# aleju/cat-generator

Hardware: AMD Instinct MI355X
Metric: images/sec per G+D step, G32up-c 32x32 RGB bs=128 per GPU (higher is better)
Workload: dtype f32

## Files before the change

### cat-generator_amd/csrc/common.h

```cpp
#pragma once
#include <hip/hip_runtime.h>
#include <algorithm>
#include <stdint.h>
#include <stdio.h>
#include <string.h>
#include "../../include/catgan.h"

namespace cg {

char* err_buf();
int fail(const char* fmt, ...);

inline hipStream_t S(void* s) { return reinterpret_cast<hipStream_t>(s); }

#define CG_HIP(call)                                                              \
    do {                                                                          \
        hipError_t e__ = (call);                                                  \
        if (e__ != hipSuccess)                                                    \
            return cg::fail("%s:%d %s -> %s", __FILE__, __LINE__, #call,          \
                            hipGetErrorString(e__));                              \
    } while (0)

#define CG_LAUNCH_CHECK()                                                         \
    do {                                                                          \
        hipError_t e__ = hipGetLastError();                                       \
        if (e__ != hipSuccess)                                                    \
            return cg::fail("%s:%d kernel launch -> %s", __FILE__, __LINE__,      \
                            hipGetErrorString(e__));                              \
    } while (0)

#define CG_REQUIRE(cond, ...)                                                     \
    do {                                                                          \
        if (!(cond)) return cg::fail(__VA_ARGS__);                                \
    } while (0)

constexpr int kNumCU = 256;

#ifndef CG_TIMING_PROBE
#define CG_TIMING_PROBE 0
#endif
#define CG_PROBE_HALF(fam, T) (((CG_TIMING_PROBE) & (fam)) ? ((T) + 1) / 2 : (T))
constexpr int kEwWgsPerCU = 4, kColReduceWgsPerCU = 1;

enum Opt {
    OPT_SKINNY, OPT_GEMM_BK32, OPT_WINO_BK, OPT_NN_TILE, OPT_TN_TILE, OPT_NN_SPLITS, OPT_TN_SPLITS,
    OPT_XCD_SWIZZLE, OPT_NN_GLDS, OPT_TN_GLDS, OPT_WINO_GLDS, OPT_PAD_SKIP, OPT_WINO3, OPT_WINO_DGRAD_FUSE, OPT_WINO_DGRAD_FUSE_LAUNCHES,
    OPT_WINO3_LAUNCHES, OPT_PACK_WIDE, OPT_SAMPLER_ATOMIC_LAUNCHES, OPT_COUNT
};
long opt(Opt o);
void opt_count(Opt o);

static inline int cdiv(long a, long b) { return (int)((a + b - 1) / b); }

constexpr size_t kColScratchBytes = 8u << 20;
void* col_scratch(hipStream_t stream);
hipStream_t queue_stream(hipStream_t ref, int cls, int slot);
int queue_class(hipStream_t ref, hipStream_t s);

constexpr int MAXG = 4;
constexpr int kMaxStridedGroups = 36;
template <typename T>
__device__ __forceinline__ T sel4(int i, T a, T b, T c, T d) { return i == 0 ? a : (i == 1 ? b : (i == 2 ? c : d)); }
__device__ __forceinline__ float4 ld4(const float* p) { return *reinterpret_cast<const float4*>(p); }
__device__ __forceinline__ float f4c(const float4& v, int i) { return i == 0 ? v.x : (i == 1 ? v.y : (i == 2 ? v.z : v.w)); }
template <typename T>
static inline void set4(T& p0, T& p1, T& p2, T& p3, const T* src, int n) {
    T* const dst[MAXG] = {&p0, &p1, &p2, &p3};
    for (int i = 0; i < MAXG; ++i) *dst[i] = (src && i < n) ? src[i] : nullptr;
}
__device__ __host__ __forceinline__ int phase_map(int a, int d, int pad) { return ((a + d - pad) >> 1) - ((a - pad) >> 1); }
static inline int phase_kp(int k, int pad) { return phase_map(0, k - 1, pad) + 1; }

struct WgradParts {
    const float* part;
    const float* bias_part;
    float* const* gw;
    float* const* gb;
    long gws;
    int ngroups, S, Cin, Cout, kH, kW, pad, ups;
    float scale;
};
int wgrad_finish(hipStream_t st, const WgradParts& w, bool defer);
void wgrad_discard_all();

constexpr int kSkinnyWgradBlocks = 512;
bool skinny_ok(int ngroups, int Cin, int Cout, int kH, int kW, int padH, int padW, int ups);
size_t skinny_wgrad_ws_bytes(int Cin, int Cout);
void skinny_valu_forward(hipStream_t st, const float* x, const float* w, const float* bias, float* y, int N, int H, int W, int Cin, int Cout);
void skinny_valu_wgrad(hipStream_t st, const float* x, const float* dy, float* part, float* bias_part, int N, int H, int W, int Cin, int Cout,
                       int blocks, long ppb);
bool skinny_mfma_ok(int Cin, int Cout, int H, int W);
int skinny_mfma_forward(hipStream_t st, const float* x, const float* w, const float* bias, float* y, int N, int H, int W, int Cin, int Cout);
int skinny_mfma_wgrad(hipStream_t st, const float* x, const float* dy, float* part, float* bias_part, int N, int H, int W, int Cin, int Cout,
                      int max_blocks);

bool head_wgrad_ok(int N, int T, int C, int Co);
int head_wgrad(hipStream_t st, const float* x, const float* dy, float* gw, float* gb, int N, int T, int C, int Co, float scale);
constexpr int kWino3UOffset = 9 * 64 * 64, kWino3UFloats = 16 * 64 * 64;
static inline bool wino3_layer(int Cout, int Cin, int kH, int kW) { return Cout == 64 && Cin == 64 && kH == 3 && kW == 3; }
bool wino3_geom_ok(int ngroups, int N, int H, int W, int Cin, int Cout, int kH, int kW, int padH, int padW, int ups);
int wino3_note_pack(hipStream_t st, int n, const float* const* w, float* const* wf, float* const* wb, const int* Cout, const int* Cin,
                    const int* kH, const int* kW, const int* wb_map);
int wino3_forward(hipStream_t st, int ngroups, const float* const* x, const float* const* wpk, const float* const* bias, float* const* y,
                  int N, int H, int W);

static inline int ew_grid(long n, int per_block = 256) {
    long b = (n + per_block - 1) / per_block;
    if (b < 1) b = 1;
    const long cap = (long)kNumCU * kEwWgsPerCU;
    if (b > cap) b = cap;
    return (int)b;
}

static inline bool al16(const void* p) { return ((uintptr_t)p & 15) == 0; }
template <class... P>
static inline bool vec_ok(long n, const P*... p) { return n % 4 == 0 && (al16(p) && ...); }
#define CG_EW_LAUNCH(kern, n, ...)                                                                    \
    do {                                                                                              \
        if ((n) > 0) {                                                                                \
            hipLaunchKernelGGL(kern, dim3(cg::ew_grid(n)), dim3(256), 0, cg::S(stream), __VA_ARGS__); \
            CG_LAUNCH_CHECK();                                                                        \
        }                                                                                             \
    } while (0)
#define CG_EW_LAUNCH_V(vec, kern, n, ...)                                                                                   \
    do {                                                                                                                    \
        if ((n) > 0) {                                                                                                      \
            if (vec) { constexpr int V = 4; hipLaunchKernelGGL(kern, dim3(cg::ew_grid((n) / V)), dim3(256), 0, cg::S(stream), __VA_ARGS__); } \
            else { constexpr int V = 1; hipLaunchKernelGGL(kern, dim3(cg::ew_grid((n) / V)), dim3(256), 0, cg::S(stream), __VA_ARGS__); }    \
            CG_LAUNCH_CHECK();                                                                                              \
        }                                                                                                                   \
    } while (0)

constexpr int tile_of_row_c(int l) {
    return ((l < 4 || (l >= 12 && l < 16) || (l >= 20 && l < 28)) ? 0 : 16) +
           ((l < 4 || (l >= 12 && l < 16) || (l >= 20 && l < 28)) ? (l < 4 ? l : (l < 16 ? l - 8 : l - 12)) : (l < 12 ? l - 4 : (l < 20 ? l - 8 : l - 16)));
}
__device__ __forceinline__ int tile_of_row(int l) {
    const bool ga = l < 4 || (l >= 12 && l < 16) || (l >= 20 && l < 28);
    const int rank = ga ? (l < 4 ? l : (l < 16 ? l - 8 : l - 12)) : (l < 12 ? l - 4 : (l < 20 ? l - 8 : l - 16));
    return (ga ? 0 : 16) + rank;
}
__device__ __forceinline__ void wino3_pack_item(const float* __restrict__ w, float* uf, float* ub, int idx) {
    constexpr int C = 64;
    const int co = idx / C, ci = idx % C;
    const float G[4][3] = {{1.f, 0.f, 0.f}, {.5f, .5f, .5f}, {.5f, -.5f, .5f}, {0.f, 0.f, 1.f}};
    for (int flip = 0; flip < 2; ++flip) {
        float* U = flip ? ub : uf;
        if (!U) continue;
        float g[3][3];
        for (int a = 0; a < 3; ++a)
            for (int b = 0; b < 3; ++b) g[a][b] = flip ? w[((long)ci * C + co) * 9 + (2 - a) * 3 + (2 - b)] : w[((long)co * C + ci) * 9 + a * 3 + b];
        float t[4][3];
        for (int i = 0; i < 4; ++i)
            for (int b = 0; b < 3; ++b) t[i][b] = G[i][0] * g[0][b] + G[i][1] * g[1][b] + G[i][2] * g[2][b];
        for (int i = 0; i < 4; ++i)
            for (int k = 0; k < 4; ++k)
                U[(((long)(i * 4 + k) * (C / 4) + ci / 4) * C + co) * 4 + (ci & 3)] = t[i][0] * G[k][0] + t[i][1] * G[k][1] + t[i][2] * G[k][2];
    }
}
__device__ __forceinline__ float u01(uint64_t seed, uint64_t ctr) {
    uint64_t z = seed + (ctr + 1) * 0x9E3779B97F4A7C15ull;
    z = (z ^ (z >> 30)) * 0xBF58476D1CE4E5B9ull;
    z = (z ^ (z >> 27)) * 0x94D049BB133111EBull;
    z = z ^ (z >> 31);
    return (float)(z >> 40) * (1.0f / 16777216.0f);
}
__device__ __forceinline__ float wave_sum(float v) {
#pragma unroll
    for (int off = 32; off > 0; off >>= 1) v += __shfl_down(v, off, 64);
    return v;
}
__device__ __forceinline__ double wave_sum(double v) {
#pragma unroll
    for (int off = 32; off > 0; off >>= 1) v += __shfl_down(v, off, 64);
    return v;
}

#ifndef CG_COL_HANDOVER
#define CG_COL_HANDOVER 3
#endif
__device__ __forceinline__ void st_agent(double* p, double v) {
#if CG_COL_HANDOVER == 4
    const unsigned long long old = __hip_atomic_exchange((unsigned long long*)p, (unsigned long long)__double_as_longlong(v),
                                                         __ATOMIC_RELAXED, __HIP_MEMORY_SCOPE_AGENT);
    asm volatile("" ::"v"(old));
#else
    __hip_atomic_store(p, v, __ATOMIC_RELAXED, __HIP_MEMORY_SCOPE_AGENT);
#endif
}
__device__ __forceinline__ double ld_agent(const double* p) {
#if CG_COL_HANDOVER == 4
    unsigned long long zero = 0ull;
    asm volatile("" : "+v"(zero));
    return __longlong_as_double((long long)__hip_atomic_fetch_or((unsigned long long*)const_cast<double*>(p), zero, __ATOMIC_RELAXED,
                                                                 __HIP_MEMORY_SCOPE_AGENT));
#else
    return __hip_atomic_load(const_cast<double*>(p), __ATOMIC_RELAXED, __HIP_MEMORY_SCOPE_AGENT);
#endif
}

__device__ __forceinline__ bool last_block_arrives(unsigned* counter, unsigned total) {
    __shared__ int last_flag;
#if CG_COL_HANDOVER == 0
    __threadfence();
#else
    asm volatile("s_waitcnt vmcnt(0)" ::: "memory");
#endif
    __syncthreads();
    if (threadIdx.x == 0) {
#if CG_COL_HANDOVER == 3
        __builtin_amdgcn_fence(__ATOMIC_RELEASE, "agent");
#endif
        const unsigned t = __hip_atomic_fetch_add(counter, 1u, __ATOMIC_RELAXED, __HIP_MEMORY_SCOPE_AGENT);
        last_flag = (t == total - 1) ? 1 : 0;
        if (last_flag) __hip_atomic_store(counter, 0u, __ATOMIC_RELAXED, __HIP_MEMORY_SCOPE_AGENT);
    }
    __syncthreads();
#if CG_COL_HANDOVER == 0
    if (last_flag) __threadfence();
#elif CG_COL_HANDOVER == 3
    if (last_flag) __builtin_amdgcn_fence(__ATOMIC_ACQUIRE, "agent");
#endif
    return last_flag != 0;
}

struct ColTree {
    int G, ngroups;
    unsigned* counters;
    double* part;
    double* grp;
    double* extra;
};
constexpr int kColTreeMaxGroups = 32;
static inline bool col_tree_layout(char* scr, long chunks, size_t nk, size_t nextra, ColTree& t) {
    t.G = (int)std::max<long>(16, (chunks + kColTreeMaxGroups - 1) / kColTreeMaxGroups);
// ... 143 lines not shown
```

### cat-generator_amd/csrc/gemm.hip

```cpp
#include "common.h"
#include <stdlib.h>
#include <algorithm>
#include <type_traits>

using cg::f4c;
using cg::kMaxStridedGroups;
using cg::ld4;
using cg::MAXG;
using cg::phase_kp;
using cg::sel4;
using cg::set4;

namespace {

typedef float f32x16 __attribute__((ext_vector_type(16)));
typedef unsigned int u32x4 __attribute__((ext_vector_type(4)));

constexpr int BK = 16;
constexpr unsigned OOB = 0x80000000u;
#ifdef CG_TRACE
__device__ unsigned long long* g_trace;
#define CG_STAMP(slot)                                                                                                  \
    do {                                                                                                                \
        if (threadIdx.x == 0 && g_trace) {                                                                              \
// ... 1286 lines not shown
    const bool fast = (g.Cin % BK == 0) && al;
    const bool vecb = (g.Cout % 4 == 0) && alw;
    const bool bk32 = cg::opt(cg::OPT_GEMM_BK32) != 0 && (g.Cin % 32 == 0) && (p.kchunk % 32 == 0);
    if (a.xcd_swizzle & 4) {
        const int ntn = cg::cdiv(g.Cout, p.tc.bn);
        const double xb = (double)(g.M / (g.Hg * g.Wg)) * g.Hs * g.Ws * g.Cin * 4.0, wb = (double)g.Ktot * g.Cout * 4.0;
        if (!(ntn == 2 || ntn == 4 || ntn == 8) || ntn * xb + (8 / ntn) * wb >= xb + 8 * wb) a.xcd_swizzle &= ~4;
    }
    if (p.pm) {
        a.g.pmn = g.M / (g.Hg * g.Wg);
        a.g.pm_lg = ilog2_exact(a.g.pmn);
    }
    dim3 grid(cg::cdiv(g.M, p.tc.bm) * cg::cdiv(g.Cout, p.tc.bn), p.splits, g.nphase * ngroups);
    with_block_tile(p.tc, [&](auto t) {
        using T = decltype(t);
        launch_nn<T::BM, T::BN, T::WM, T::WN>(a, grid, st, fast, vecb, bk32);
    });
    CG_LAUNCH_CHECK();
    if (p.splits > 1) {
        const long PMN = (long)ngroups * g.nphase * g.M * g.Cout;
        bool v4 = g.Cout % 4 == 0 && (uintptr_t)ws % 16 == 0;
        for (int i = 0; i < ngroups; ++i)
            v4 = v4 && (uintptr_t)y[i] % 16 == 0 && (!bias || (uintptr_t)bias[i] % 16 == 0) && (!a.act || (uintptr_t)ep->y_act[i] % 16 == 0);
        if ((PMN >= 256L * 1024 || p.splits < 8) && v4)
            hipLaunchKernelGGL((nn_splitk_reduce_kernel<1, true>), dim3(cg::ew_grid(PMN / 4)), dim3(256), 0, st, a, p.splits);
        else if (PMN >= 256L * 1024 || p.splits < 8)
            hipLaunchKernelGGL(nn_splitk_reduce_kernel<1>, dim3(cg::ew_grid(PMN)), dim3(256), 0, st, a, p.splits);
        else
            hipLaunchKernelGGL(nn_splitk_reduce_kernel<8>, dim3((unsigned)cg::cdiv(PMN, 32)), dim3(256), 0, st, a, p.splits);
        CG_LAUNCH_CHECK();
    }
    return 0;
}

static int conv_geom(Geom& g, int N, int Hp, int Wp, int Cin, int Cout, int kH, int kW, int padH, int padW, int ups) {
    if (check_dims(N, Hp, Wp, Cin, Cout, kH, kW, padH, padW, ups)) return 1;
    return ups ? geom_phase_fwd(g, N, Hp, Wp, Cin, Cout, kH, padH) : geom_plain(g, N, Hp, Wp, Cin, Cout, kH, kW, padH, padW);
}

}

#ifdef CG_TRACE
extern "C" int cg_debug_set_trace(void* p) {
    unsigned long long* q = (unsigned long long*)p;
    return hipMemcpyToSymbol(HIP_SYMBOL(g_trace), &q, sizeof(q)) == hipSuccess ? 0 : 1;
}
#endif

extern "C" {

size_t cg_conv2d_workspace_bytes_grouped(int ngroups, int N, int Hp, int Wp, int Cin, int Cout, int kH, int kW, int padH,
                                         int padW, int ups) {
    Geom g;
    if (ngroups < 1 || ngroups > MAXG || conv_geom(g, N, Hp, Wp, Cin, Cout, kH, kW, padH, padW, ups)) return 0;
    return nn_ws_bytes(g, plan_nn(g, ngroups), ngroups);
}
size_t cg_conv2d_workspace_bytes(int N, int Hp, int Wp, int Cin, int Cout, int kH, int kW, int padH, int padW, int ups) {
    return cg_conv2d_workspace_bytes_grouped(1, N, Hp, Wp, Cin, Cout, kH, kW, padH, padW, ups);
}

size_t cg_conv2d_stats_rows(int N, int Hp, int Wp, int Cin, int Cout, int kH, int kW, int padH, int padW, int ups) {
    Geom g;
    if (conv_geom(g, N, Hp, Wp, Cin, Cout, kH, kW, padH, padW, ups)) return 0;
    if (cg::skinny_ok(1, Cin, Cout, kH, kW, padH, padW, ups)) return 0;
    const NNPlan p = plan_nn(g, 1, false);
    if (p.splits != 1) return 0;
    const int wm = p.tc.bn == 32 ? 4 : 2;
    return (size_t)g.nphase * cg::cdiv(g.M, p.tc.bm) * wm;
}

int cg_conv2d_forward_ex(void* stream, int ngroups, const float* const* x, const float* const* wpk, const float* const* bias,
                         float* const* y, int N, int Hp, int Wp, int Cin, int Cout, int kH, int kW, int padH, int padW,
                         int ups, int act, float slope, const float* const* alpha, float* const* y_act, float* stats,
                         void* ws, size_t ws_bytes) {
    CG_REQUIRE(x && wpk && y, "cg_conv2d_forward_ex: null pointer");
    Geom g;
    if (conv_geom(g, N, Hp, Wp, Cin, Cout, kH, kW, padH, padW, ups)) return 1;
    CG_REQUIRE(!cg::skinny_ok(ngroups, Cin, Cout, kH, kW, padH, padW, ups) || (act == 0 && !stats),
               "cg_conv2d_forward_ex: no fused epilogue on the skinny (<= 4 output planes) path");
    if (act == 0 && !stats)
        return cg_conv2d_forward_grouped(stream, ngroups, x, wpk, bias, y, N, Hp, Wp, Cin, Cout, kH, kW, padH, padW, ups, ws,
                                         ws_bytes);
    Epi ep{act, slope, alpha, y_act, stats};
    return run_nn(cg::S(stream), g, ngroups, x, wpk, bias, y, ws, ws_bytes, "cg_conv2d_forward_ex", &ep);
}

int cg_conv2d_forward_grouped(void* stream, int ngroups, const float* const* x, const float* const* wpk,
                              const float* const* bias, float* const* y, int N, int Hp, int Wp, int Cin, int Cout, int kH,
                              int kW, int padH, int padW, int ups, void* ws, size_t ws_bytes) {
    CG_REQUIRE(x && wpk && y, "cg_conv2d_forward_grouped: null pointer");
    Geom g;
    if (conv_geom(g, N, Hp, Wp, Cin, Cout, kH, kW, padH, padW, ups)) return 1;
    if (cg::skinny_ok(ngroups, Cin, Cout, kH, kW, padH, padW, ups) && x[0] && wpk[0] && y[0] && (uintptr_t)x[0] % 16 == 0 &&
        (long)N * Hp * Wp < 0x7fffffffL) {
        const float* b0 = bias ? bias[0] : nullptr;
        if (cg::opt(cg::OPT_SKINNY) == 1 && cg::skinny_mfma_ok(Cin, Cout, Hp, Wp)) {
            if (cg::skinny_mfma_forward(cg::S(stream), x[0], wpk[0], b0, y[0], N, Hp, Wp, Cin, Cout)) return 1;
        }
        else cg::skinny_valu_forward(cg::S(stream), x[0], wpk[0], b0, y[0], N, Hp, Wp, Cin, Cout);
        CG_LAUNCH_CHECK();
        return 0;
    }
    if (cg::wino3_geom_ok(ngroups, N, Hp, Wp, Cin, Cout, kH, kW, padH, padW, ups)) {
        const int rc = cg::wino3_forward(cg::S(stream), ngroups, x, wpk, bias, y, N, Hp, Wp);
        if (rc) return rc < 0 ? 1 : 0;
    }
    return run_nn(cg::S(stream), g, ngroups, x, wpk, bias, y, ws, ws_bytes, "cg_conv2d_forward_grouped");
}

int cg_conv2d_forward(void* stream, const float* x, const float* wpk, const float* bias, float* y, int N, int Hp, int Wp,
                      int Cin, int Cout, int kH, int kW, int padH, int padW, int ups, void* ws, size_t ws_bytes) {
    return cg_conv2d_forward_grouped(stream, 1, &x, &wpk, bias ? &bias : nullptr, &y, N, Hp, Wp, Cin, Cout, kH, kW, padH, padW,
                                     ups, ws, ws_bytes);
}

size_t cg_conv2d_dgrad_ups2_workspace_bytes(int N, int Hp, int Wp, int Cin, int Cout, int k, int pad) {
    Geom g;
    if (check_dims(N, Hp, Wp, Cin, Cout, k, k, pad, pad, 1)) return 0;
    if (geom_phase_dgrad(g, N, Hp, Wp, Cin, Cout, k, pad)) return 0;
    return nn_ws_bytes(g, plan_nn(g, 1), 1);
}

int cg_conv2d_dgrad_ups2(void* stream, const float* dy, const float* wb_ph, float* dx_lo, int N, int Hp, int Wp, int Cin,
                         int Cout, int k, int pad, void* ws, size_t ws_bytes) {
    CG_REQUIRE(dy && wb_ph && dx_lo, "cg_conv2d_dgrad_ups2: null pointer");
    Geom g;
    if (check_dims(N, Hp, Wp, Cin, Cout, k, k, pad, pad, 1)) return 1;
    if (geom_phase_dgrad(g, N, Hp, Wp, Cin, Cout, k, pad)) return 1;
    return run_nn(cg::S(stream), g, 1, &dy, &wb_ph, nullptr, &dx_lo, ws, ws_bytes, "cg_conv2d_dgrad_ups2");
}

static size_t wgrad_ws_bytes_groups(int ngroups, int maxg, int N, int Hp, int Wp, int Cin, int Cout, int kH, int kW, int padH, int padW, int ups) {
    Geom g;
    if (ngroups < 1 || ngroups > maxg || conv_geom(g, N, Hp, Wp, Cin, Cout, kH, kW, padH, padW, ups)) return 0;
    const size_t reg = tn_ws_bytes(g, plan_tn(g, ngroups), ngroups);
    return cg::skinny_ok(ngroups, Cin, Cout, kH, kW, padH, padW, ups) ? std::max(reg, cg::skinny_wgrad_ws_bytes(Cin, Cout)) : reg;
}
size_t cg_conv2d_wgrad_workspace_bytes_grouped(int ngroups, int N, int Hp, int Wp, int Cin, int Cout, int kH, int kW,
                                               int padH, int padW, int ups) {
    return wgrad_ws_bytes_groups(ngroups, MAXG, N, Hp, Wp, Cin, Cout, kH, kW, padH, padW, ups);
}
size_t cg_conv2d_wgrad_workspace_bytes_strided(int ngroups, int N, int Hp, int Wp, int Cin, int Cout, int kH, int kW,
                                               int padH, int padW, int ups) {
    return wgrad_ws_bytes_groups(ngroups, kMaxStridedGroups, N, Hp, Wp, Cin, Cout, kH, kW, padH, padW, ups);
}
size_t cg_conv2d_wgrad_workspace_bytes(int N, int Hp, int Wp, int Cin, int Cout, int kH, int kW, int padH, int padW,
                                       int ups) {
    return cg_conv2d_wgrad_workspace_bytes_grouped(1, N, Hp, Wp, Cin, Cout, kH, kW, padH, padW, ups);
}

namespace {
int wgrad_impl(void* stream, int ngroups, const float* const* x, const float* const* dy, float* const* gw, float* const* gb, int N,
               int Hp, int Wp, int Cin, int Cout, int kH, int kW, int padH, int padW, int ups, float scale, void* ws, size_t ws_bytes,
               bool defer, long xgs = 0, long dgs = 0, long gws = 0, bool gemm_only = false);
}

int cg_conv2d_wgrad_grouped(void* stream, int ngroups, const float* const* x, const float* const* dy, float* const* gw,
                            float* const* gb, int N, int Hp, int Wp, int Cin, int Cout, int kH, int kW, int padH, int padW,
                            int ups, float scale, void* ws, size_t ws_bytes) {
    return wgrad_impl(stream, ngroups, x, dy, gw, gb, N, Hp, Wp, Cin, Cout, kH, kW, padH, padW, ups, scale, ws, ws_bytes, false);
}

int cg_conv2d_wgrad_grouped_deferred(void* stream, int ngroups, const float* const* x, const float* const* dy, float* const* gw,
                                     float* const* gb, int N, int Hp, int Wp, int Cin, int Cout, int kH, int kW, int padH, int padW,
                                     int ups, float scale, void* ws, size_t ws_bytes) {
    return wgrad_impl(stream, ngroups, x, dy, gw, gb, N, Hp, Wp, Cin, Cout, kH, kW, padH, padW, ups, scale, ws, ws_bytes, true);
}

int cg_conv2d_wgrad_strided(void* stream, int ngroups, const float* x, long x_stride, const float* dy, long dy_stride, float* gw,
                            long gw_stride, int N, int Hp, int Wp, int Cin, int Cout, int kH, int kW, int padH, int padW, int ups,
                            float scale, void* ws, size_t ws_bytes) {
    CG_REQUIRE(x && dy && gw && x_stride > 0 && dy_stride > 0 && gw_stride > 0, "cg_conv2d_wgrad_strided: bad arguments");
    CG_REQUIRE(ngroups >= 1 && ngroups <= kMaxStridedGroups, "cg_conv2d_wgrad_strided: 1..%d groups per launch", kMaxStridedGroups);
    return wgrad_impl(stream, ngroups, &x, &dy, &gw, nullptr, N, Hp, Wp, Cin, Cout, kH, kW, padH, padW, ups, scale, ws, ws_bytes, false,
                      x_stride, dy_stride, gw_stride);
}

int cg_conv2d_wgrad_gemm(void* stream, const float* x, const float* dy, int N, int Hp, int Wp, int Cin, int Cout, int kH, int kW, int padH,
                         int padW, int ups, void* ws, size_t ws_bytes) {
    CG_REQUIRE(x && dy && ws, "cg_conv2d_wgrad_gemm: null pointer");
    CG_REQUIRE(!cg::skinny_ok(1, Cin, Cout, kH, kW, padH, padW, ups), "cg_conv2d_wgrad_gemm: this geometry runs the skinny kernel, not the GEMM");
    float* gw = (float*)ws;
    return wgrad_impl(stream, 1, &x, &dy, &gw, nullptr, N, Hp, Wp, Cin, Cout, kH, kW, padH, padW, ups, 1.f, ws, ws_bytes, false, 0, 0, 0, true);
}

namespace {
void launch_tn_tile(const TNArgs& a, const TileCfg& tc, bool tng, dim3 grid, hipStream_t st, bool veca, bool vecb) {
    with_block_tile(tc, [&](auto t) {
        using T = decltype(t);
        if (tng) launch_tng<T::BM, T::BN, T::WM, T::WN>(a, grid, st);
        else launch_tn<T::BM, T::BN, T::WM, T::WN>(a, grid, st, veca, vecb);
    });
}

int wgrad_impl(void* stream, int ngroups, const float* const* x, const float* const* dy, float* const* gw, float* const* gb, int N,
               int Hp, int Wp, int Cin, int Cout, int kH, int kW, int padH, int padW, int ups, float scale, void* ws, size_t ws_bytes,
               bool defer, long xgs, long dgs, long gws_, bool gemm_only) {
    CG_REQUIRE(x && dy && gw, "cg_conv2d_wgrad: null pointer");
    const bool strided = xgs != 0;
    CG_REQUIRE(ngroups >= 1 && ngroups <= (strided ? kMaxStridedGroups : MAXG), "cg_conv2d_wgrad: 1..%d groups per launch", strided ? kMaxStridedGroups : MAXG);
    CG_REQUIRE(!strided || (!gb && !defer), "cg_conv2d_wgrad: strided groups carry no bias gradient and are not deferred");
    TNArgs a;
    memset(&a, 0, sizeof(a));
    if (conv_geom(a.g, N, Hp, Wp, Cin, Cout, kH, kW, padH, padW, ups)) return 1;
    const Geom& g = a.g;
    if (!strided && cg::skinny_ok(ngroups, Cin, Cout, kH, kW, padH, padW, ups) && x[0] && dy[0] && gw[0] && (uintptr_t)x[0] % 16 == 0 && ws &&
        ws_bytes >= cg::skinny_wgrad_ws_bytes(Cin, Cout) && (long)N * Hp * Wp < 0x7fffffffL) {
        hipStream_t st = cg::S(stream);
        const long npix = (long)N * Hp * Wp;
        const long ppb = (npix + cg::kSkinnyWgradBlocks - 1) / cg::kSkinnyWgradBlocks;
        int blocks = (int)((npix + ppb - 1) / ppb);
        float* part = (float*)ws;
        float* bpart = part + (size_t)cg::kSkinnyWgradBlocks * 9 * Cin * Cout;
        float* gb0 = gb ? gb[0] : nullptr;
        if (cg::opt(cg::OPT_SKINNY) == 1 && cg::skinny_mfma_ok(Cin, Cout, Hp, Wp)) {
            blocks = cg::skinny_mfma_wgrad(st, x[0], dy[0], part, gb0 ? bpart : nullptr, N, Hp, Wp, Cin, Cout, cg::kSkinnyWgradBlocks / 2);
            if (blocks < 0) return 1;
        }
        else cg::skinny_valu_wgrad(st, x[0], dy[0], part, gb0 ? bpart : nullptr, N, Hp, Wp, Cin, Cout, blocks, ppb);
        CG_LAUNCH_CHECK();
        const cg::WgradParts parts{part, gb0 ? bpart : nullptr, gw, gb, 0, 1, blocks, Cin, Cout, 3, 3, 1, 0, scale};
        return cg::wgrad_finish(st, parts, defer);
    }
    if (!strided && !gemm_only && ngroups == 1 && !ups && kH == Hp && kW == Wp && padH == 0 && padW == 0 && cg::opt(cg::OPT_PAD_SKIP) > 0 &&
        cg::opt(cg::OPT_TN_GLDS) && cg::head_wgrad_ok(N, kH * kW, Cin, Cout) && x[0] && dy[0] && gw[0] && (uintptr_t)x[0] % 16 == 0 &&
        (uintptr_t)dy[0] % 16 == 0 && (uintptr_t)gw[0] % 4 == 0)
        return cg::head_wgrad(cg::S(stream), x[0], dy[0], gw[0], gb ? gb[0] : nullptr, N, kH * kW, Cin, Cout, scale) != 0;
    TNPlan p = plan_tn(g, ngroups);
    const size_t need = tn_ws_bytes(g, p, ngroups);
    CG_REQUIRE(ws && ws_bytes >= need, "cg_conv2d_wgrad: workspace too small (%zu < %zu)", ws_bytes, need);
    const int nptr = strided ? 1 : ngroups;
    bool veca = Cin % 4 == 0, vecb = Cout % 4 == 0, any_gb = false;
    for (int i = 0; i < nptr; ++i) {
        CG_REQUIRE(x[i] && dy[i] && gw[i], "cg_conv2d_wgrad: null pointer (group %d)", i);
        veca = veca && ((uintptr_t)x[i] % 16 == 0);
        vecb = vecb && ((uintptr_t)dy[i] % 16 == 0);
        any_gb = any_gb || (gb && gb[i]);
    }
    if (strided) { veca = veca && xgs % 4 == 0; vecb = vecb && dgs % 4 == 0; }
    if (p.pm && !(veca && vecb)) p = plan_tn(g, ngroups, false);
    a.xgs = xgs; a.dgs = dgs;
    set4(a.x0, a.x1, a.x2, a.x3, x, nptr);
    set4(a.d0, a.d1, a.d2, a.d3, dy, nptr);
    a.ngroups = ngroups; a.part = (float*)ws; a.pchunk = p.pchunk;
    a.xcd_swizzle = (int)cg::opt(cg::OPT_XCD_SWIZZLE);
    const int ZP = ngroups * g.nphase;
    const long wplane = (long)g.Ktot * g.Cout;
    a.bias_part = any_gb ? (float*)ws + (size_t)p.splits * ZP * wplane : nullptr;
    hipStream_t st = cg::S(stream);
    dim3 grid(cg::cdiv(g.Ktot, p.tc.bm) * cg::cdiv(g.Cout, p.tc.bn), p.splits, ZP);
    if (p.pm && veca && vecb) a.pm_n = g.M / (g.Hg * g.Wg);
    launch_tn_tile(a, p.tc, a.pm_n || tng_ok(g, p.pchunk, veca, vecb), grid, st, veca, vecb);
    CG_LAUNCH_CHECK();
    if (gemm_only) return 0;
    const cg::WgradParts parts{(const float*)ws, a.bias_part, gw, gb, strided ? gws_ : 0, ngroups, p.splits, Cin, Cout, kH, kW, padH, ups, scale};
    return cg::wgrad_finish(st, parts, defer);
}

}

int cg_conv2d_wgrad(void* stream, const float* x, const float* dy, float* gw, float* gb, int N, int Hp, int Wp, int Cin,
                    int Cout, int kH, int kW, int padH, int padW, int ups, float scale, void* ws, size_t ws_bytes) {
    CG_REQUIRE(x && dy && gw, "cg_conv2d_wgrad: null pointer");
    return cg_conv2d_wgrad_grouped(stream, 1, &x, &dy, &gw, &gb, N, Hp, Wp, Cin, Cout, kH, kW, padH, padW, ups, scale, ws,
                                   ws_bytes);
}

}
```

### cat-generator_amd/csrc/net.hip

```cpp
#include "net_plan.h"
#include "net_compiler.h"

namespace cg { extern unsigned long g_opt_epoch; }

namespace {

Net* NET(void* h) { return reinterpret_cast<Net*>(h); }

long param_numel(const Mod& m, int slot) {
    switch (m.kind) {
        case K_LINEAR: return slot == 0 ? m.ia[0] * m.ia[1] : m.ia[1];
        case K_CONV: return slot == 0 ? m.ia[0] * m.ia[1] * m.ia[2] * m.ia[3] : m.ia[1];
        case K_PRELU: return slot == 0 ? 1 : 0;
        case K_BN: return m.ia[0];
        default: return 0;
    }
}
void collect_params(Net* n, const Mod& m, vector<std::pair<float*, long>>& out) {
    if (m.gw) out.push_back({m.gw, param_numel(m, 0)});
    if (m.gb) out.push_back({m.gb, param_numel(m, 1)});
    for (int c : m.kids) collect_params(n, *n->mods[c], out);
}

int settle_allocs(Net* n) {
// ... 51 lines not shown
    for (Op& op : ops) {
        if (at++ == join_before) {
            if (n->trace) trace_note(n, "event|wait|packs|all");
            else
                for (int t = 0; t < c.pr->nstreams; ++t)
                    if (t != 1 && hipStreamWaitEvent(c.st[t], n->pack_ev, 0) != hipSuccess) { g_cur_net = nullptr; return cg::fail("cg_net: hipStreamWaitEvent failed"); }
        }
        c.cur = op.sidx;
        const int rc = op.fn(c);
        if (rc) { g_cur_net = nullptr; cg::wgrad_discard_all(); return rc; }
    }
    g_cur_net = nullptr;
    return 0;
}

int sync_packs(Net* n, Prog* pr, Run& c, int* join_before) {
    *join_before = -1;
    if (n->params_dirty) {
        for (auto& mp : n->mods) { mp->dirty_plain = true; mp->dirty_ups = true; }
        n->params_dirty = false;
    }
    void* stream = c.S(0);
    vector<const float*> w; vector<float*> wf, wb; vector<int> co, ci, kh, kw, mp_;
    vector<Mod*> ups;
    g_cur_net = n;
    for (auto& up : n->mods) {
        Mod& m = *up;
        if (!m.is_gemm()) continue;
        if (m.wf && m.dirty_plain) {
            if (!m.w) return cg::fail("cg_net: layer %d has no weight bound (cg_net_bind)", m.id);
            w.push_back(m.w); wf.push_back(m.wf); wb.push_back(m.wb);
            if (m.pk_map == 1) { co.push_back((int)m.ia[1]); ci.push_back((int)m.map_c); kh.push_back((int)m.map_h); kw.push_back((int)m.map_w); mp_.push_back(1); }
            else if (m.kind == K_LINEAR) { co.push_back((int)m.ia[1]); ci.push_back((int)m.ia[0]); kh.push_back(1); kw.push_back(1); mp_.push_back(0); }
            else { co.push_back((int)m.ia[1]); ci.push_back((int)m.ia[0]); kh.push_back((int)m.kH()); kw.push_back((int)m.kW()); mp_.push_back(0); }
            m.dirty_plain = false;
        }
        if (m.wf_ph && m.dirty_ups) ups.push_back(&m);
    }
    if (!w.empty() && n->K->pack_conv_weight_batch(stream, (int)w.size(), w.data(), wf.data(), wb.data(), co.data(), ci.data(), kh.data(), kw.data(), mp_.data())) return 1;
    auto first_op = [&](const Mod* m) { auto it = pr->ups_first_op.find(m->id); return it == pr->ups_first_op.end() ? -1 : it->second; };
    std::stable_sort(ups.begin(), ups.end(), [&](const Mod* a, const Mod* b) { return first_op(a) < first_op(b); });
    const bool can_side = n->pack_overlap && c.st[1] != c.st[0];
    bool forked = false;
    for (size_t i = 0; i < ups.size(); ++i) {
        Mod& m = *ups[i];
        const int fo = first_op(&m);
        const bool on_side = can_side && i >= 1 && fo > 0 && fo < (int)pr->fwd.size();
        if (on_side && !forked) {
            forked = true;
            if (n->trace) trace_note(n, "event|record|packs_fork|s0\nevent|wait|packs_fork|s1");
            else if (hipEventRecord(n->pack_fork_ev, c.st[0]) != hipSuccess || hipStreamWaitEvent(c.st[1], n->pack_fork_ev, 0) != hipSuccess)
                return cg::fail("cg_net: cannot fork the packing stream");
        }
        void* st = on_side ? c.S(1) : stream;
        if (n->K->pack_conv_weight_ups2(st, m.w, m.wf_ph, m.wb_ph, (int)m.ia[1], (int)m.ia[0], (int)m.kH(), (int)((m.kH() - 1) / 2))) return 1;
        if (m.wino && n->K->conv2d_ups2_wino_pack(st, m.wf_ph, m.wb_ph, m.u_fwd, m.u_bwd, (int)m.ia[1], (int)m.ia[0])) return 1;
        if (m.u22 && n->K->conv2d_ups2_wino22_pack(st, m.wf_ph, m.wb_ph, m.u22, m.u22b, (int)m.ia[1], (int)m.ia[0])) return 1;
        if (on_side && (*join_before < 0 || fo < *join_before)) *join_before = fo;
        m.dirty_ups = false;
    }
    if (forked) {
        if (n->trace) trace_note(n, "event|record|packs|s1");
        else if (hipEventRecord(n->pack_ev, c.st[1]) != hipSuccess) return cg::fail("cg_net: hipEventRecord failed");
        n->pack_inflight = true;
    } else if ((!w.empty() || !ups.empty()) && !n->trace) {
        if (hipEventRecord(n->pack_ev, c.st[0]) != hipSuccess) return cg::fail("cg_net: hipEventRecord failed");
        n->pack_inflight = true;
    }
    g_cur_net = nullptr;
    return 0;
}

std::string prog_key(Net* n, int nd, const long* dims, int fmt) {
    std::string k = std::to_string(fmt) + ":";
    for (int i = 0; i < nd; ++i) k += std::to_string(dims[i]) + "x";
    k += "|t";
    for (auto& m : n->mods) if (m->kind == K_BN || m->kind == K_SDROP || m->kind == K_DROP) k += m->train ? '1' : '0';
    k += "|w" + std::to_string(n->world) + (n->sync_bn ? "s" : "-") + (n->bucket_overlap ? "b" : "-");
    k += "|o" + std::to_string(n->overlap_groups) + std::to_string(n->defer_wgrad) + std::to_string(n->winograd) + std::to_string(n->fusion) +
         std::to_string(n->stacking) + std::to_string(n->grouped) + std::to_string(n->share_pool) + std::to_string(n->sampler_shared) +
         std::to_string(n->view_fuse) + std::to_string(n->cat_fuse) + std::to_string(n->fuse_locnet) + std::to_string(n->head_fuse) +
         std::to_string(n->wgrad_stream) + std::to_string(n->wino22) + std::to_string(n->wino_dsplit) + "m" +
         std::to_string(n->wino_min_tiles);
    return k;
}

int forward_plan(Net* n, void* stream, int nd, const long* dims, int fmt, Prog** out) {
    const std::string key = prog_key(n, nd, dims, fmt);
    auto it = n->progs.find(key);
    if (it != n->progs.end() && it->second->opt_epoch != cg::g_opt_epoch) {
        if (n->last == it->second.get()) n->last = nullptr;
        n->progs.erase(it); it = n->progs.end();
    }
    if (it == n->progs.end()) {
        std::unique_ptr<Prog> pr(new Prog());
        pr->net = n; pr->opt_epoch = cg::g_opt_epoch;
        Val in; in.none = false; in.ext = EXT_X; in.nd = nd; for (int i = 0; i < nd; ++i) in.d[i] = dims[i]; in.fmt = fmt;
        pr->in = in;
        Compiler C(n, pr.get());
        C.ops = &pr->fwd;
        Compiler::GCtx ctx{{C.rng}};
        pr->out = C.gfwd({n->mods[0].get()}, {in}, ctx)[0];
        if (C.failed) return cg::fail("%s", n->err);
        CG_REQUIRE(!pr->out.is_tab, "cg_net_forward: the root module returns a table");
        pr->out = C.materialise(pr->out);
        pr->draws = ctx.cur[0];
        if (ensure_streams(n, std::max(pr->nstreams, n->pack_overlap && pr->ups_first_op.size() >= 2 ? 2 : 1), stream)) return 1;
        if (settle_allocs(n)) return 1;
        it = n->progs.emplace(key, std::move(pr)).first;
    }
    *out = it->second.get();
    return 0;
}

void make_buckets(Net* n, Prog* pr) {
    const Mod& root = *n->mods[0];
    bool contiguous = true; float* expect = nullptr;
    for (size_t i = 0; i < root.kids.size(); ++i) {
        vector<std::pair<float*, long>> ps;
        collect_params(n, *n->mods[root.kids[i]], ps);
        long cnt = 0; for (auto& p : ps) cnt += p.second;
        if (n->mods[root.kids[i]]->is_gemm() || pr->buckets.empty()) {
            if (ps.empty() && pr->buckets.empty()) continue;
            pr->buckets.push_back({ps.empty() ? expect : ps[0].first, 0}); pr->bucket_first.push_back((int)i);
        }
        for (auto& p : ps) { if (expect && p.first != expect) contiguous = false; expect = p.first + p.second; }
        pr->buckets.back().second += cnt;
    }
    if (!contiguous) { pr->buckets.clear(); pr->bucket_first.clear(); }
    constexpr long kMinBucket = 65536;
    vector<std::pair<float*, long>> mb; vector<int> mf;
    long accn = 0;
    for (int j = (int)pr->buckets.size() - 1; j >= 0; --j) {
        accn += pr->buckets[j].second;
        if (accn >= kMinBucket || j == 0) {
            mb.insert(mb.begin(), {pr->buckets[j].first, accn}); mf.insert(mf.begin(), pr->bucket_first[j]);
            accn = 0;
        }
    }
    pr->buckets.swap(mb); pr->bucket_first.swap(mf);
}

int compile_backward(Net* n, Prog* pr, void* stream, int acc, int gy_fmt) {
    Compiler C(n, pr);
    C.ops = &pr->bwd[acc];
    C.acc_pass = acc != 0;
    pr->bwd[acc].clear();
    Mod& root = *n->mods[0];
    if (acc && n->bucket_overlap && n->world > 1 && root.kind == K_SEQ && root.kids.size() > 1 && pr->buckets.empty()) make_buckets(n, pr);
    C.bucket_done_upto = (int)root.kids.size();
    Val go = pr->out; go.ext = EXT_GY; go.off = 0; go.p = nullptr; go.fmt = gy_fmt; go.blk = 0; go.gi = go.gc = 0;
    Val gi = C.gbwd({&root}, {pr->in}, {go}, acc != 0, true)[0];
    if (C.failed) return cg::fail("%s", n->err);
    if (acc) { C.buckets_start(); C.flush_wgrad(); C.wg_join_all(); }
    CG_REQUIRE(!gi.is_tab, "cg_net_backward: the root module's gradInput is a table");
    pr->gin[acc] = gi;
    pr->have_bwd[acc] = true;
    if (ensure_streams(n, pr->nstreams, stream)) return 1;
    return settle_allocs(n);
}

void put_val(const Val& v, float* p, int fmt, float** ptr, int* nd, long* dims, int* fmtp) {
    if (ptr) *ptr = p;
    if (nd) *nd = v.nd;
    if (dims) for (int i = 0; i < 4; ++i) dims[i] = v.d[i];
    if (fmtp) *fmtp = fmt;
}

}

extern "C" {

int cg_net_create(void** net) {
    CG_REQUIRE(net, "cg_net_create: null pointer");
    Net* n = new Net();
    *net = n;
    if (const char* e = getenv("CG_NET_OPTIONS")) {
        std::string all(e);
        size_t pos = 0;
        while (pos < all.size()) {
            size_t end = all.find(',', pos);
            if (end == std::string::npos) end = all.size();
            const std::string kv = all.substr(pos, end - pos);
            const size_t eq = kv.find('=');
            if (eq == std::string::npos || eq == 0) { delete n; *net = nullptr; return cg::fail("CG_NET_OPTIONS: expected name=value, got '%s'", kv.c_str()); }
            if (cg_net_set_option(n, kv.substr(0, eq).c_str(), atol(kv.c_str() + eq + 1))) { delete n; *net = nullptr; return 1; }
            pos = end + 1;
        }
    }
    return 0;
}

int cg_net_destroy(void* net) {
    Net* n = NET(net);
    if (!n) return 0;
    for (void* p : n->owned) { if (n->trace) free(p); else (void)hipFree(p); }
    for (auto e : n->side_ev) (void)hipEventDestroy(e);
    if (n->fork_ev) (void)hipEventDestroy(n->fork_ev);
    if (n->pack_ev) { (void)hipEventDestroy(n->pack_fork_ev); (void)hipEventDestroy(n->pack_ev); }
    if (n->pair_fork_ev) { (void)hipEventDestroy(n->pair_fork_ev); (void)hipEventDestroy(n->pair_a_ev); (void)hipEventDestroy(n->pair_join_ev); }
    for (int t = 0; t < 4; ++t) if (n->wg_fork_ev[t]) { (void)hipEventDestroy(n->wg_fork_ev[t]); (void)hipEventDestroy(n->wg_join_ev[t]); }
    delete n;
    return 0;
}

int cg_net_set_option(void* net, const char* name, long value) {
    Net* n = NET(net);
    CG_REQUIRE(n && name, "cg_net_set_option: null pointer");
    struct { const char* nm; int* p; } tab[] = {
        {"overlap_groups", &n->overlap_groups}, {"defer_wgrad", &n->defer_wgrad}, {"winograd", &n->winograd}, {"share_pool", &n->share_pool},
        {"sampler_shared", &n->sampler_shared}, {"view_fuse", &n->view_fuse}, {"cat_fuse", &n->cat_fuse}, {"stacking", &n->stacking},
        {"grouped", &n->grouped}, {"fusion", &n->fusion}, {"fuse_locnet", &n->fuse_locnet}, {"pack_overlap", &n->pack_overlap},
        {"head_fuse", &n->head_fuse}, {"wgrad_stream", &n->wgrad_stream}, {"wino_dsplit", &n->wino_dsplit}};
    if (!strcmp(name, "trace")) {
        CG_REQUIRE(n->progs.empty(), "cg_net_set_option: trace must be chosen before the first pass");
        n->trace = value != 0; n->K = n->trace ? &kTraceTable : &kRealTable;
        return 0;
    }
    if (!strcmp(name, "defer_running")) { n->defer_running = value != 0; return 0; }
    if (!strcmp(name, "winograd_min_tiles")) { n->wino_min_tiles = value; return 0; }
    if (!strcmp(name, "winograd22")) { n->wino22 = (int)value & 3; return 0; }
    if (!strcmp(name, "fuse_locnet")) { n->fuse_locnet = (int)value; return 0; }
    for (auto& t : tab) if (!strcmp(name, t.nm)) { *t.p = value != 0; return 0; }
    return cg::fail("cg_net_set_option: unknown option %s", name);
}

int cg_net_set_allocator(void* net, cg_alloc_fn alloc, void* user) {
    Net* n = NET(net);
    CG_REQUIRE(n, "cg_net_set_allocator: null net");
    n->alloc_fn = alloc; n->alloc_user = user;
    return 0;
}

int cg_net_set_hook(void* net, cg_hook_fn hook, void* user) {
    Net* n = NET(net);
    CG_REQUIRE(n, "cg_net_set_hook: null net");
    n->hook = hook; n->hook_user = user;
    return 0;
}

int cg_net_set_dp(void* net, int world, int sync_bn, void* comm_bn, void* comm_grad, int bucket_overlap) {
    Net* n = NET(net);
    CG_REQUIRE(n && world >= 1, "cg_net_set_dp: bad arguments");
    n->world = world; n->sync_bn = sync_bn != 0; n->comm_bn = comm_bn; n->comm_grad = comm_grad; n->bucket_overlap = (bucket_overlap & 1) != 0;
    n->hook_too = (bucket_overlap & 2) != 0;
    return 0;
}

int cg_net_add(void* net, int parent, int kind, const long* iargs, int niargs, const float* fargs, int nfargs, int* id) {
    Net* n = NET(net);
    CG_REQUIRE(n && id, "cg_net_add: null pointer");
    CG_REQUIRE(kind >= 0 && kind < K_COUNT, "cg_net_add: unknown module kind %d", kind);
    CG_REQUIRE(niargs <= 8 && nfargs <= 4, "cg_net_add: too many arguments");
    CG_REQUIRE(parent < (int)n->mods.size(), "cg_net_add: unknown parent %d", parent);
    CG_REQUIRE((parent < 0) == n->mods.empty(), "cg_net_add: exactly the first module is the root (parent -1)");
    if (parent >= 0) CG_REQUIRE(n->mods[parent]->is_container(), "cg_net_add: parent %d is not a container", parent);
    std::unique_ptr<Mod> m(new Mod());
    m->id = (int)n->mods.size(); m->kind = kind; m->parent = parent;
    for (int i = 0; i < niargs; ++i) m->ia[i] = iargs[i];
    for (int i = 0; i < nfargs; ++i) m->fa[i] = fargs[i];
    if (kind == K_VIEW) m->ia[7] = niargs;
    if (kind == K_CONV) CG_REQUIRE(m->ia[6] <= 1 && m->ia[7] <= 1, "cg_net_add: only stride 1 convolutions are on the path");
    if (kind == K_CONCAT) CG_REQUIRE(m->ia[0] == 2, "cg_net_add: nn.Concat joins on dimension 2 (channels)");
    if (parent >= 0) n->mods[parent]->kids.push_back(m->id);
    *id = m->id;
    n->mods.push_back(std::move(m));
    n->progs.clear(); n->last = nullptr;
    return 0;
}

int cg_net_bind(void* net, int id, int slot, float* param, float* grad) {
    Net* n = NET(net);
    CG_REQUIRE(n && id >= 0 && id < (int)n->mods.size(), "cg_net_bind: unknown module %d", id);
    Mod& m = *n->mods[id];
    if (slot == 0) { m.w = param; m.gw = grad; }
    else if (slot == 1) { m.b = param; m.gb = grad; }
    else if (slot == 2) { m.rmean = param; m.rvar = grad; }
    else return cg::fail("cg_net_bind: slot %d (0 weight, 1 bias, 2 running mean / var)", slot);
    n->params_dirty = true;
    for (auto& kv : n->progs) { kv.second->buckets.clear(); kv.second->bucket_first.clear(); kv.second->have_bwd[1] = false; kv.second->bwd[1].clear(); }
    return 0;
}

int cg_net_set_training(void* net, int id, int train) {
    Net* n = NET(net);
    CG_REQUIRE(n && id < (int)n->mods.size(), "cg_net_set_training: unknown module %d", id);
    if (id < 0) for (auto& m : n->mods) m->train = train != 0;
    else n->mods[id]->train = train != 0;
    return 0;
}

int cg_net_params_changed(void* net) {
    Net* n = NET(net);
    CG_REQUIRE(n, "cg_net_params_changed: null net");
    n->params_dirty = true;
    return 0;
}

int cg_net_trace_region(void* net, const void* base, size_t bytes) {
    Net* n = NET(net);
    CG_REQUIRE(n && base, "cg_net_trace_region: null pointer");
    n->regions.push_back(Region{(const char*)base, bytes});
    return 0;
}

int cg_net_trace_take(void* net, char* out, size_t cap, size_t* len) {
    Net* n = NET(net);
// ... 168 lines not shown
```

### cat-generator_amd/csrc/net_compiler.h

```cpp
#pragma once

namespace {

struct Compiler {
    struct GCtx { vector<long> cur; };

    struct Prep { Val x; int wsel; Val out; Geo g; bool ok = true; };
    enum { W_PLAIN_F = 0, W_PH_F, W_PLAIN_B, W_PH_B, W_CANON };
    static float* wsel(const Mod* m, int sel) {
        switch (sel) {
            case W_PLAIN_F: return m->wf;
            case W_PH_F: return m->wf_ph;
            case W_PLAIN_B: return m->wb ? m->wb : m->w;
            case W_PH_B: return m->wb_ph;
            default: return m->w;
        }
    }

    Net* net;
    Prog* pr;
    vector<Op>* ops = nullptr;
    int cs = 0;
    long rng = 0;
    int dry = 0;
    bool failed = false;
    int pend[8] = {0, 0, 0, 0, 0, 0, 0, 0};
    bool wg_used[4] = {false, false, false, false};
    bool wg_unjoined[4] = {false, false, false, false};
    bool acc_pass = false;

    Compiler(Net* n, Prog* p) : net(n), pr(p) {}
    const KTable* K() const { return net->K; }
    Mod& M(int id) { return *net->mods[id]; }
    MS& S(const Mod& m) { return pr->ms[m.id]; }
    int err(const char* fmt, ...) {
        va_list ap; va_start(ap, fmt); vsnprintf(net->err, sizeof net->err, fmt, ap); va_end(ap);
        failed = true;
        return 1;
    }

    void* alloc(size_t bytes) {
        if (dry) return nullptr;
        bytes = (bytes + 255) & ~(size_t)255;
        if (bytes == 0) bytes = 256;
        void* p = nullptr;
        if (net->trace) {
            p = calloc(1, bytes);
        } else if (net->alloc_fn) {
            p = net->alloc_fn(net->alloc_user, bytes);
        } else {
            if (hipMalloc(&p, bytes) != hipSuccess || hipMemset(p, 0, bytes) != hipSuccess) p = nullptr;
            else net->fresh_allocs = true;
        }
        if (!p) { err("cg_net: allocation of %zu bytes failed", bytes); return nullptr; }
        if (!net->alloc_fn || net->trace) net->owned.push_back(p);
        net->regions.push_back(Region{(const char*)p, bytes});
        return p;
    }
    Val anon(std::initializer_list<long> dims, int fmt = PLAIN) {
        long n = 1; for (long x : dims) n *= x;
        Val v = mkval((float*)alloc((size_t)n * 4), dims, fmt);
        return v;
    }
    Val anon_like(const Val& x, int fmt) {
        Val v = x; v.p = (float*)alloc((size_t)x.numel() * 4); v.ext = 0; v.off = 0; v.fmt = fmt; v.ups = 0; v.blk = 0; v.gi = v.gc = 0;
        return v;
    }
    Val buf(const Mod& m, const std::string& role, std::initializer_list<long> dims, int fmt = PLAIN, size_t elem = 4) {
        long n = 1; for (long x : dims) n *= x;
        std::string key = role + "#" + std::to_string(n);
        MS& s = S(m);
        auto it = s.bufs.find(key);
        if (it == s.bufs.end()) {
            Val v = mkval((float*)alloc((size_t)n * elem), dims, fmt);
            s.bufs[key] = v;
            return v;
        }
        Val& b = it->second;
        Val want = mkval(nullptr, dims, fmt);
        if (!b.same_shape(want) || b.fmt != fmt) {
            const bool keep = want.nd && b.nd && want.d[0] == b.d[0];
            Val nb = reshape(b, dims, fmt, 0, keep);
            b = nb;
        }
        return b;
    }
    Val buf_like(const Mod& m, const std::string& role, const Val& like, int fmt) {
        switch (like.nd) {
            case 1: return buf(m, role, {like.d[0]}, fmt);
            case 2: return buf(m, role, {like.d[0], like.d[1]}, fmt);
            case 3: return buf(m, role, {like.d[0], like.d[1], like.d[2]}, fmt);
            default: return buf(m, role, {like.d[0], like.d[1], like.d[2], like.d[3]}, fmt);
        }
    }
    void ws_need(size_t bytes) {
        if (dry) return;
        if (bytes < 4096) bytes = 4096;
        if ((int)pr->ws.size() <= cs) { pr->ws.resize(cs + 1, nullptr); pr->ws_bytes.resize(cs + 1, 0); }
        if (pr->ws_bytes[cs] < bytes) {
            size_t nb = bytes + bytes / 4;
            pr->ws[cs] = alloc(nb);
            pr->ws_bytes[cs] = nb;
        }
    }
    template <class F> void emit(F f) {
        if (dry) return;
        ops->push_back(Op{cs, std::function<int(Run&)>(f)});
    }
    void use_stream(int sidx) { if (!dry && sidx + 1 > pr->nstreams) pr->nstreams = sidx + 1; }

    Val materialise(const Val& x) {
        if (!x.ups) return x;
        long N = x.d[0], C = x.d[1], H = x.d[2], W = x.d[3];
        Val out = anon({N, C, H, W}, NHWC);
        const KTable* k = K();
        emit([=](Run& c) { return k->upsample2x_forward(c.CS(), c.P(x), c.P(out), (int)N, (int)(H >> 1), (int)(W >> 1), (int)C); });
        return out;
    }

    Val as_nhwc(const Val& x, bool keep_ups = false) {
        if (x.fmt == NHWC) return (keep_ups || !x.ups) ? x : materialise(x);
        if (x.nd != 4) { err("cg_net: expected a 4-D feature map"); return x; }
        long N = x.d[0], C = x.d[1], H = x.d[2], W = x.d[3];
        Val out = anon({N, C, H, W}, NHWC);
        const KTable* k = K();
        emit([=](Run& c) { return k->nchw_to_nhwc(c.CS(), c.P(x), c.P(out), (int)N, (int)C, (int)H, (int)W); });
        return out;
    }
    Val as_plain(const Val& x0) {
        if (x0.fmt == PLAIN) return x0;
        Val x = materialise(x0);
        long N = x.d[0], C = x.d[1], H = x.d[2], W = x.d[3];
        Val out = anon({N, C, H, W}, PLAIN);
        const KTable* k = K();
        emit([=](Run& c) { return k->nhwc_to_nchw(c.CS(), c.P(x), c.P(out), (int)N, (int)C, (int)H, (int)W); });
        return out;
    }
    void emit_scaled_copy(const Val& dst, const Val& src, float f) {
        const KTable* k = K();
        const long n = src.phys();
        emit([=](Run& c) { return k->memcpy_d2d(c.CS(), c.P(dst), c.P(src), (size_t)n * 4); });
        emit([=](Run& c) { return k->scale(c.CS(), c.P(dst), f, n); });
    }
    Val match_fmt(const Val& g, const Val& like) {
        if (g.fmt == like.fmt) return g;
        return like.fmt == NHWC ? as_nhwc(g) : as_plain(g);
    }

    vector<Val> split(const Val& Y, int G) {
        vector<Val> out;
        const long n = Y.phys() / G, N = Y.d[0] / G;
        for (int i = 0; i < G; ++i) {
            Val v = Y.at((size_t)i * n * 4);
            v.d[0] = N; v.blk = Y.key(); v.gi = i; v.gc = G;
            out.push_back(v);
        }
        return out;
    }
    bool stacked(const vector<Val>& xs, Val* out) {
        if (xs.empty() || xs[0].is_tab || xs[0].none || !xs[0].blk || xs[0].gc != (int)xs.size()) return false;
        const Val& x0 = xs[0];
        for (size_t i = 0; i < xs.size(); ++i) {
            const Val& x = xs[i];
            if (x.is_tab || x.none || x.blk != x0.blk || x.gi != (int)i || !x.same_shape(x0) || x.fmt != x0.fmt || x.ups) return false;
        }
        if (out) {
            Val b = x0;
            b.d[0] = x0.d[0] * (long)xs.size(); b.blk = 0; b.gi = b.gc = 0;
            *out = b;
        }
        return true;
    }
    void seed_slices(const vector<Mod*>& mods, const std::string& role, const Val& shape_of, int fmt) {
        const int G = (int)mods.size();
        const long n = shape_of.numel();
        std::string key = role + "#" + std::to_string(n);
        vector<Val> cur; bool all = true;
        for (Mod* m : mods) {
            auto it = S(*m).bufs.find(key);
            if (it == S(*m).bufs.end() || !it->second.same_shape(shape_of) || it->second.fmt != fmt) { all = false; break; }
            cur.push_back(it->second);
        }
        if (all && stacked(cur, nullptr)) return;
        Val bs = shape_of; bs.d[0] *= G;
        Val block = buf_like(*mods[0], role + ".block", bs, fmt);
        vector<Val> sl = split(block, G);
        for (int i = 0; i < G; ++i) S(*mods[i]).bufs[key] = sl[i];
    }
    Val restack(const Mod& owner, vector<Val> xs, const Val& like) {
        for (auto& x : xs) x = match_fmt(x, like);
        Val bs = xs[0]; bs.d[0] *= (long)xs.size(); bs.ups = 0;
        Val block = buf_like(owner, "restack.block", bs, xs[0].fmt);
        const size_t nb = (size_t)xs[0].phys() * 4;
        const KTable* k = K();
        for (size_t i = 0; i < xs.size(); ++i) {
            Val dst = block.at(i * nb), src = xs[i];
            emit([=](Run& c) { return k->memcpy_d2d(c.CS(), c.P(dst), c.P(src), nb); });
        }
        return block;
    }

    void need_plain(Mod& m, bool map, long C = 0, long H = 0, long W = 0) {
        if (dry) return;
        const size_t n = cg_pack_conv_weight_floats((int)m.ia[1], (int)m.ia[0], (int)m.kH(), (int)m.kW());
        const long taps = map ? H * W : m.kH() * m.kW();
        const int want = map ? 1 : 0;
        if (m.pk_map == want && (!map || (m.map_c == C && m.map_h == H && m.map_w == W))) return;
        if (!m.wf) m.wf = (float*)alloc(n * 4);
        if (taps > 1 && !m.wb) m.wb = (float*)alloc(n * 4);
        if (taps <= 1) m.wb = nullptr;
        m.pk_map = want; m.map_c = C; m.map_h = H; m.map_w = W;
        m.dirty_plain = true;
    }
    void need_ups(Mod& m, bool wino) {
        if (dry) return;
        if (ops == &pr->fwd && !pr->ups_first_op.count(m.id)) pr->ups_first_op[m.id] = (int)ops->size();
        if (!m.wf_ph) {
            const size_t n = cg_pack_conv_weight_ups2_floats((int)m.ia[1], (int)m.ia[0], (int)m.kH(), (int)((m.kH() - 1) / 2));
            m.wf_ph = (float*)alloc(n * 4); m.wb_ph = (float*)alloc(n * 4);
            m.dirty_ups = true;
        }
        if (wino && !m.wino) {
            m.wino = true;
            const size_t nu = cg_conv2d_ups2_wino_u_floats((int)m.ia[0], (int)m.ia[1]);
            m.u_fwd = (float*)alloc(nu * 4); m.u_bwd = (float*)alloc(nu * 4);
            m.dirty_ups = true;
        }
    }

    static bool can_fold_ups(const Mod& m) { return m.kH() == m.kW() && m.kH() % 2 == 1 && m.padH() == m.padW() && m.padH() == (m.kH() - 1) / 2; }
    bool use_wino22(Mod& m, const Val& x) {
        if (!(net->winograd && (net->wino22 & 1) && m.kind == K_CONV && x.ups && m.kH() == 3 && m.kW() == 3 && m.padH() == 1 && m.padW() == 1)) return false;
        const long N = x.d[0], Hp = x.d[2] >> 1, Wp = x.d[3] >> 1;
        if (N * Hp * Wp / 4 < net->wino_min_tiles) return false;
        return cg_conv2d_ups2_wino22_supported((int)N, (int)Hp, (int)Wp, (int)m.ia[0], (int)m.ia[1]) != 0;
    }
    bool use_wino(Mod& m, const Val& x) {
        if (!(net->winograd && m.kind == K_CONV && x.ups && m.kH() == 5 && m.kW() == 5 && m.padH() == 2 && m.padW() == 2)) return false;
        const long N = x.d[0], Hp = x.d[2] >> 1, Wp = x.d[3] >> 1;
        if (N * Hp * Wp / 4 < net->wino_min_tiles) return false;
        return cg_conv2d_ups2_wino_supported((int)N, (int)Hp, (int)Wp, (int)m.ia[0], (int)m.ia[1], 5, 2) != 0;
    }
    static bool epilogue_ok(const Geo& g) {
        const bool skinny = g.ups == 0 && g.kH == 3 && g.kW == 3 && g.padH == 1 && g.padW == 1 && (g.Cout == 1 || g.Cout == 3) &&
                            (g.Cin == 64 || g.Cin == 128);
        return !skinny;
    }
    Prep prep_fwd(Mod& m, const Val& in) {
        Prep p;
        MS& s = S(m);
        if (m.kind == K_LINEAR) {
            Val x = in;
            const long o = m.ia[1];
            if (s.map_in && !(x.nd == 4 && x.fmt == NHWC && !x.ups && x.d[1] == s.mc && x.d[2] == s.mh && x.d[3] == s.mw)) s.map_in = false;
            if (s.map_in) {
                const long N = x.d[0];
                need_plain(m, true, s.mc, s.mh, s.mw);
                p.x = x; p.wsel = W_PLAIN_F; p.out = buf(m, "out", {N, o});
                p.g = Geo{(int)N, (int)s.mh, (int)s.mw, (int)s.mc, (int)o, (int)s.mh, (int)s.mw, 0, 0, 0};
                return p;
            }
            x = as_plain(x);
            const long N = x.d[0], i = x.numel() / x.d[0];
            need_plain(m, false);
            p.x = x; p.wsel = W_PLAIN_F; p.out = buf(m, "out", {N, o});
            p.g = Geo{(int)N, 1, 1, (int)i, (int)o, 1, 1, 0, 0, 0};
            return p;
        }
        Val x = as_nhwc(in, true);
        if (x.ups && !can_fold_ups(m)) x = materialise(x);
        const long N = x.d[0], H = x.d[2], W = x.d[3];
        const long Hp = H >> x.ups, Wp = W >> x.ups, Ho = H + 2 * m.padH() - m.kH() + 1, Wo = W + 2 * m.padW() - m.kW() + 1;
        if (x.d[1] != m.ia[0]) { err("cg_net: convolution %d got %ld input planes, expects %ld", m.id, x.d[1], m.ia[0]); }
        if (x.ups) { need_ups(m, false); p.wsel = W_PH_F; } else { need_plain(m, false); p.wsel = W_PLAIN_F; }
        p.x = x;
        p.out = buf(m, "out", {N, m.ia[1], Ho, Wo}, NHWC);
        p.g = Geo{(int)N, (int)Hp, (int)Wp, (int)m.ia[0], (int)m.ia[1], (int)m.kH(), (int)m.kW(), (int)m.padH(), (int)m.padW(), x.ups};
        return p;
    }
    Prep prep_gin(Mod& m, const Val& go) {
        Prep p;
        MS& s = S(m);
        if (m.kind == K_LINEAR) {
            Val dy = as_plain(go);
            const long N = dy.d[0], o = dy.numel() / dy.d[0], i = m.ia[0];
            p.x = dy;
            if (s.map_in) {
                p.wsel = W_PLAIN_B; p.out = buf(m, "gin", {N, s.mc, s.mh, s.mw}, NHWC);
            } else {
                p.wsel = W_CANON; p.out = buf(m, "gin", {N, i});
            }
            p.g = Geo{(int)N, 1, 1, (int)o, (int)i, 1, 1, 0, 0, 0};
            return p;
        }
        const Val& x = s.x;
        if (x.ups) { p.ok = false; return p; }
        Val dy = as_nhwc(go);
        const long N = dy.d[0], Ho = dy.d[2], Wo = dy.d[3];
        p.x = dy; p.wsel = W_PLAIN_B;
        p.out = buf(m, "gin", {N, m.ia[0], x.d[2], x.d[3]}, NHWC);
        p.g = Geo{(int)N, (int)Ho, (int)Wo, (int)m.ia[1], (int)m.ia[0], (int)m.kH(), (int)m.kW(), (int)(m.kH() - 1 - m.padH()),
                  (int)(m.kW() - 1 - m.padW()), 0};
        return p;
    }
    struct PrepAcc { Val x, dy; Geo g; };
    PrepAcc prep_acc(Mod& m, const Val& go) {
        PrepAcc p;
        MS& s = S(m);
        p.x = s.x;
        if (m.kind == K_LINEAR) {
            p.dy = as_plain(go);
            if (s.map_in) p.g = Geo{(int)p.x.d[0], (int)s.mh, (int)s.mw, (int)s.mc, (int)m.ia[1], (int)s.mh, (int)s.mw, 0, 0, 0};
            else p.g = Geo{(int)p.x.d[0], 1, 1, (int)(p.x.numel() / p.x.d[0]), (int)m.ia[1], 1, 1, 0, 0, 0};
            return p;
        }
        p.dy = as_nhwc(go);
        const Val& x = s.x;
        p.g = Geo{(int)x.d[0], (int)(x.d[2] >> x.ups), (int)(x.d[3] >> x.ups), (int)m.ia[0], (int)m.ia[1], (int)m.kH(), (int)m.kW(),
                  (int)m.padH(), (int)m.padW(), x.ups};
        return p;
    }

    bool prep_group(const vector<Mod*>& mods, const vector<Val>& ins, Prep (Compiler::*prep)(Mod&, const Val&), const char* role, bool epilogue,
                    vector<Prep>& preps) {
        const int G = (int)mods.size();
        for (int b = 0; b < G; ++b) preps.push_back((this->*prep)(*mods[b], ins[b]));
        bool ok = G <= 4, wino = false;
        for (int b = 0; b < G; ++b) {
            ok = ok && preps[b].ok && (!epilogue || epilogue_ok(preps[b].g));
            wino = wino || (ok && mods[b]->kind == K_CONV && preps[b].x.ups && use_wino(*mods[b], preps[b].x));
        }
        for (int b = 1; ok && b < G; ++b) ok = preps[b].g == preps[0].g;
        if (!ok || wino) return false;
        vector<Val> outs; for (auto& p : preps) outs.push_back(p.out);
        if (G > 1 && net->stacking && !stacked(outs, nullptr)) {
            seed_slices(mods, role, preps[0].out, preps[0].out.fmt);
            preps.clear();
            for (int b = 0; b < G; ++b) preps.push_back((this->*prep)(*mods[b], ins[b]));
        }
        return true;
    }
    struct Epi { vector<Mod*> acts; vector<Val> ya; Val part; };
    void emit_gemm(const vector<Mod*>& mods, const vector<Prep>& preps, const Epi& e, bool bias = true) {
        const KTable* k = K();
        const int G = (int)mods.size();
        const Geo g = preps[0].g;
        ws_need(cg_conv2d_workspace_bytes_grouped(G, GEO(g)));
        if (e.acts.empty() && e.part.none) {
            if (G == 1) {
                const Prep p = preps[0]; Mod* mp = mods[0];
                emit([=](Run& c) { return k->conv2d_forward(c.CS(), c.P(p.x), wsel(mp, p.wsel), bias ? mp->b : nullptr, c.P(p.out), GEO(p.g), c.W(), c.WB()); });
                return;
            }
            emit([=](Run& c) {
                const float *x[4], *w[4], *bi[4]; float* y[4];
                for (int b = 0; b < G; ++b) { x[b] = c.P(preps[b].x); w[b] = wsel(mods[b], preps[b].wsel); bi[b] = mods[b]->b; y[b] = c.P(preps[b].out); }
                return k->conv2d_forward_grouped(c.CS(), G, x, w, bias ? bi : nullptr, y, GEO(g), c.W(), c.WB());
            });
            return;
        }
        const int code = e.acts.empty() ? 0 : e.acts[0]->kind == K_PRELU ? 1 : 2;
        const float slope = code == 2 ? e.acts[0]->fa[0] : 0.f;
        const vector<Mod*> ac = e.acts; const vector<Val> ys = e.ya; const Val part = e.part;
        emit([=](Run& c) {
            const float *x[4], *w[4], *bi[4], *al[4]; float *y[4], *ya[4];
            for (int b = 0; b < G; ++b) {
                x[b] = c.P(preps[b].x); w[b] = wsel(mods[b], preps[b].wsel); bi[b] = mods[b]->b; y[b] = c.P(preps[b].out);
                if (code) { al[b] = ac[b]->w; ya[b] = c.P(ys[b]); }
            }
            return k->conv2d_forward_ex(c.CS(), G, x, w, bi, y, GEO(g), code, slope, code == 1 ? al : nullptr, code ? ya : nullptr, c.P(part), c.W(), c.WB());
        });
    }
    vector<Val> fwd_gemm(const vector<Mod*>& mods, const vector<Prep>& preps, const Epi& e) {
        emit_gemm(mods, preps, e);
        vector<Val> outs;
        for (size_t b = 0; b < mods.size(); ++b) {
            MS& s = S(*mods[b]);
            s.x = preps[b].x; s.out = preps[b].out; s.use_wino = false; s.use_wino22 = false;
            outs.push_back(preps[b].out);
        }
        return outs;
    }
    bool defer_wg() const { return net->defer_wgrad && net->fusion; }
    void emit_wgrad_group(const vector<Mod*>& mods, const vector<PrepAcc>& ap, void*& ws, size_t& ws_bytes) {
        const KTable* k = K();
        const int G = (int)mods.size();
        const Geo g = ap[0].g;
        const bool defer = defer_wg();
        const size_t need = std::max<size_t>(cg_conv2d_wgrad_workspace_bytes_grouped(G, GEO(g)), 4096);
        if (defer) {
            if (!dry && ws_bytes < need) { ws = alloc(need); ws_bytes = need; }
            if (!dry) pend[cs]++;
        } else ws_need(need);
        void* wsp = ws; const size_t wsb = ws_bytes;
        emit([=](Run& c) {
            const float *x[4], *d_[4]; float *gw[4], *gb[4];
            for (int b = 0; b < G; ++b) { x[b] = c.P(ap[b].x); d_[b] = c.P(ap[b].dy); gw[b] = mods[b]->gw; gb[b] = mods[b]->gb; }
            if (defer) return k->conv2d_wgrad_grouped_deferred(c.CS(), G, x, d_, gw, gb, GEO(g), c.scale, wsp, wsb);
            return k->conv2d_wgrad_grouped(c.CS(), G, x, d_, gw, gb, GEO(g), c.scale, c.W(), c.WB());
        });
    }

    Val fwd(Mod& m, const Val& in) {
        Val out = fwd_launches(m, in);
        S(m).out = out;
        return out;
    }
    Val fwd_launches(Mod& m, const Val& in) {
        const KTable* k = K();
        MS& s = S(m);
        switch (m.kind) {
        case K_CONCAT: return fwd_concat(m, in);
        case K_LINEAR: case K_CONV: {
            if (m.kind == K_CONV) {
                Val x = as_nhwc(in, true);
                if (use_wino(m, x)) return fwd_wino(m, x, nullptr, nullptr);
            }
            vector<Prep> preps;
            prep_group({&m}, {in}, &Compiler::prep_fwd, "out", false, preps);
            return fwd_gemm({&m}, preps, Epi())[0];
        }
        case K_PRELU: {
            Val x = materialise(in);
            Val out = buf_like(m, "out", x, x.fmt);
            const long n = x.phys(); Mod* mp = &m;
            emit([=](Run& c) { return k->prelu_forward(c.CS(), c.P(x), mp->w, c.P(out), n); });
            s.x = x;
            return out;
        }
        case K_LRELU: {
            Val x = materialise(in);
            Val out = buf_like(m, "out", x, x.fmt);
            const long n = x.phys(); const float sl = m.fa[0];
            emit([=](Run& c) { return k->leakyrelu_forward(c.CS(), c.P(x), c.P(out), sl, n); });
            s.x = x;
            return out;
        }
        case K_SIGMOID: {
            Val x = materialise(in);
            Val out = buf_like(m, "out", x, x.fmt);
            const long n = x.phys();
            emit([=](Run& c) { return k->sigmoid_forward(c.CS(), c.P(x), c.P(out), n); });
            return out;
        }
        case K_BN: {
            Val x = as_nhwc(in);
            Val out;
            if (!m.train) {
                const long N = x.d[0], C = x.d[1], H = x.d[2], W = x.d[3], Mr = N * H * W;
                out = buf(m, "out", {N, C, H, W}, NHWC);
                Mod* mp = &m; const float eps = m.fa[0];
                emit([=](Run& c) { return k->bn_forward_eval(c.CS(), c.P(x), c.P(out), mp->w, mp->b, mp->rmean, mp->rvar, Mr, (int)C, eps); });
            } else {
                out = fwd_bn_train(m, nullptr, x, Stats());
            }
            s.x = x; s.bn_fused = false;
            return out;
        }
        case K_VIEW: {
            s.skip = false;
            Val x = as_plain(in);
            const long N = x.d[0];
            s.in_nd = x.nd; for (int i = 0; i < 4; ++i) s.in_shape[i] = x.d[i];
            Val out;
            if (m.ia[7] == 3) {
                const long C = m.ia[0], H = m.ia[1], W = m.ia[2];
                out = buf(m, "out", {N, C, H, W}, NHWC);
                emit([=](Run& c) { return k->nchw_to_nhwc(c.CS(), c.P(x), c.P(out), (int)N, (int)C, (int)H, (int)W); });
            } else {
                out = reshape(x, {N, m.ia[0]}, PLAIN);
            }
            return out;
        }
        case K_COPY: return in;
        case K_TRANSPOSE: {
            Val out;
            if (m.ia[0] == 0) {
                Val x = as_nhwc(in);
                out = reshape(x, {x.d[0], x.d[2], x.d[3], x.d[1]}, PLAIN, 0, true);
            } else {
                if (in.fmt != PLAIN) err("cg_net: nn.Transpose BHWD->NCHW expects a plain tensor");
                out = reshape(in, {in.d[0], in.d[3], in.d[1], in.d[2]}, NHWC, 0, true);
            }
            return out;
        }
        case K_UPS: {
            Val x = as_nhwc(in);
            Val out = reshape(x, {x.d[0], x.d[1], 2 * x.d[2], 2 * x.d[3]}, NHWC, 1);
            return out;
        }
        case K_AVGPOOL: case K_MAXPOOL: {
            Val x = as_nhwc(in);
            const long N = x.d[0], C = x.d[1], H = x.d[2], W = x.d[3];
            Val out = buf(m, "out", {N, C, H / 2, W / 2}, NHWC);
            const bool mx = m.kind == K_MAXPOOL;
            emit([=](Run& c) { return (mx ? k->maxpool2_forward : k->avgpool2_forward)(c.CS(), c.P(x), c.P(out), (int)N, (int)H, (int)W, (int)C); });
            s.x = x;
            return out;
        }
        case K_SDROP: {
            Val x = as_nhwc(in);
            const long N = x.d[0], C = x.d[1], H = x.d[2], W = x.d[3];
            Val out = buf(m, "out", {N, C, H, W}, NHWC);
            const float p = m.fa[0];
            if (m.train) {
                Val noise = draw_masks(m, "noise", 1, N, C, &rng, false);
                emit([=](Run& c) { return k->mask_mul(c.CS(), c.P(x), c.P(noise), c.P(out), (int)N, H * W, (int)C, 1); });
                s.noise = noise;
            } else {
                emit_scaled_copy(out, x, 1.0f - p);
            }
            return out;
        }
        case K_DROP: {
            Val x = materialise(in);
            if (!m.train) return x;
            const long n = x.phys(); const float p = m.fa[0];
            Val noise = buf_like(m, "noise", x, x.fmt), out = buf_like(m, "out", x, x.fmt);
            const long off = rng; rng += n;
            emit([=](Run& c) { return k->rng_bernoulli_dev(c.CS(), c.P(noise), n, 1.0f - p, 1.0f / (1.0f - p), c.seed, c.roff + (uint64_t)off, c.rbase); });
            emit([=](Run& c) { return k->mask_mul(c.CS(), c.P(x), c.P(noise), c.P(out), 1, n, 1, 0); });
            s.noise = noise;
            return out;
        }
        case K_AFFMAT: {
            Val p = as_plain(in);
            const long N = p.d[0];
            Val out = buf(m, "out", {N, 2, 3});
            const int r = (int)m.ia[0], sc = (int)m.ia[1], tr = (int)m.ia[2];
            emit([=](Run& c) { return k->affine_matrix_forward(c.CS(), c.P(p), c.P(out), (int)N, r, sc, tr); });
            s.p = p;
            return out;
        }
        case K_AFFGRID: {
            const long N = in.d[0], H = m.ia[0], W = m.ia[1];
            Val out = buf(m, "out", {N, H, W, 2});
            Val T = in;
            emit([=](Run& c) { return k->affine_grid_forward(c.CS(), c.P(T), c.P(out), (int)N, (int)H, (int)W); });
            return out;
        }
        case K_SAMPLER: {
            if (!in.is_tab || in.tab.size() != 2) { err("cg_net: nn.BilinearSamplerBHWD expects {images, grids}"); return in; }
            Val img = in.tab[0], grid = in.tab[1];
            if (img.fmt != PLAIN || grid.fmt != PLAIN) err("cg_net: sampler inputs must be BHWD tensors");
            const long N = img.d[0], Hi = img.d[1], Wi = img.d[2], C = img.d[3], Ho = grid.d[1], Wo = grid.d[2];
            Val out = buf(m, "out", {N, Ho, Wo, C});
            emit([=](Run& c) { return k->bilinear_sampler_forward(c.CS(), c.P(img), c.P(grid), c.P(out), (int)N, (int)Hi, (int)Wi, (int)C, (int)Ho, (int)Wo); });
            s.in_img = img; s.in_grid = grid; s.has_shared = false;
            return out;
        }
// ... 315 lines not shown
            vector<Val> cur = xs;
            for (auto& colm : chain) cur = gfwd(colm, cur, ctx);
            return cur;
        }
        const int code = a0.kind == K_PRELU ? 1 : 2;
        const float slope = code == 1 ? 0.f : a0.fa[0];
        Mod& last = d0 ? *d0 : p0;
        Val out = buf(last, "out.fused", {G * N, C, H / 2, W / 2}, NHWC);
        Val mask; bool have_mask = false;
        if (d0) { mask = draw_masks(*d0, "noise.block", G, N, C, ctx.cur.data(), true); have_mask = true; }
        const int pool_max = p0.kind == K_MAXPOOL ? 1 : 0;
        vector<Mod*> ac = acts;
        emit([=](Run& c) {
            const float* al[4];
            for (int b = 0; b < G; ++b) al[b] = ac[b]->w;
            return k->act_pool2_mask_forward(c.CS(), c.P(X), c.P(out), have_mask ? c.P(mask) : nullptr, G, (int)N, (int)H, (int)W, (int)C, code, slope,
                                             code == 1 ? al : nullptr, pool_max);
        });
        vector<Val> outs = slices(out, G), masks;
        if (have_mask) masks = slices(mask, G);
        for (int b = 0; b < G; ++b) {
            MS& sa = S(*acts[b]); sa.x = xs[b]; sa.out = Val();
            MS& sp = S(*pools[b]); sp.x = Val(); sp.out = d0 ? Val() : outs[b];
            if (d0) { MS& sd = S(*drops[b]); sd.noise = masks[b]; sd.out = outs[b]; }
        }
        MS& s0 = S(a0);
        s0.fused = true; s0.fG = G; s0.fX = X; s0.fmask = have_mask ? mask : Val(); s0.fN = N; s0.fC = C; s0.fH = H; s0.fW = W;
        return outs;
    }

    Val fwd_gemm_bn_act(Mod& conv, Mod& bn, Mod& act, const Val& in) {
        const KTable* k = K();
        Val x = as_nhwc(in, true);
        const long C = conv.ia[1];
        if (C % 4 != 0) { S(bn).bn_fused = false; return fwd(act, fwd(bn, fwd(conv, in))); }
        Stats st; Val out;
        Mod* cp = &conv;
        if (use_wino(conv, x)) {
            out = fwd_wino(conv, x, &bn, &st);
        } else if (use_wino22(conv, x)) {
            Prep p = prep_fwd(conv, x);
            const long N = x.d[0], Hp = x.d[2] >> 1, Wp = x.d[3] >> 1, Ci = conv.ia[0];
            if (!dry && !conv.u22) {
                conv.u22 = (float*)alloc(cg_conv2d_ups2_wino22_u_floats((int)Ci, (int)C) * 4);
                conv.u22b = (float*)alloc(cg_conv2d_ups2_wino22_u_floats((int)Ci, (int)C) * 4);
                conv.dirty_ups = true;
            }
            out = p.out;
            Val v = buf(conv, "wino22_v", {(long)cg_conv2d_ups2_wino22_v_floats((int)N, (int)Hp, (int)Wp, (int)Ci)});
            st.rows = (long)cg_conv2d_ups2_wino_stats_rows((int)N, (int)Hp, (int)Wp, (int)Ci, (int)C);
            if (st.rows) st.part = buf(bn, "stats_part", {st.rows, 2, C});
            const Val px = p.x, part = st.part;
            emit([=](Run& c) { return k->conv2d_ups2_wino22_forward_stats(c.CS(), c.P(px), cp->u22, cp->b, c.P(out), c.P(v), (int)N, (int)Hp, (int)Wp, (int)Ci, (int)C,
                                                                         c.P(part)); });
            S(conv).x = p.x; S(conv).out = p.out; S(conv).use_wino = false; S(conv).use_wino22 = true;
        } else {
            vector<Prep> preps;
            prep_group({&conv}, {x}, &Compiler::prep_fwd, "out", false, preps);
            st.rows = epilogue_ok(preps[0].g) ? (long)cg_conv2d_stats_rows(GEO(preps[0].g)) : 0;
            if (st.rows) st.part = buf(bn, "stats_part", {st.rows, 2, C});
            out = fwd_gemm({&conv}, preps, Epi{{}, {}, st.part})[0];
        }
        Val y = fwd_bn_train(bn, &act, out, st);
        const long Mr = out.d[0] * out.d[2] * out.d[3];
        MS& sb = S(bn); sb.x = out; sb.out = Val(); sb.bn_fused = true; sb.bnM = Mr; sb.bnC = C;
        MS& sa = S(act); sa.x = Val(); sa.out = y;
        return y;
    }

    struct LocDesc { Mod *conv1, *conv2, *lin1, *lin2; int S, Cin, P, ur, us, ut, Hg, Wg; float slope; };
    bool match_loc(Mod& q, const Val& in, LocDesc& d) {
        if (!net->fuse_locnet || !net->fusion || q.kind != K_SEQ || q.kids.size() != 3) return false;
        Mod& L = M(q.kids[0]);
        static const int want[10] = {K_AVGPOOL, K_CONV, K_LRELU, K_CONV, K_LRELU, K_AVGPOOL, K_VIEW, K_LINEAR, K_LRELU, K_LINEAR};
        if (L.kind != K_SEQ || L.kids.size() != 10 || M(q.kids[1]).kind != K_AFFMAT || M(q.kids[2]).kind != K_AFFGRID) return false;
        for (int i = 0; i < 10; ++i) if (M(L.kids[i]).kind != want[i]) return false;
        if (in.is_tab || in.none || in.nd != 4 || in.fmt != NHWC || in.ups || in.d[2] != in.d[3] || in.d[2] % 4) return false;
        d.conv1 = &M(L.kids[1]); d.conv2 = &M(L.kids[3]); d.lin1 = &M(L.kids[7]); d.lin2 = &M(L.kids[9]);
        d.S = (int)(in.d[2] / 2); d.Cin = (int)in.d[1]; d.P = (int)d.lin2->ia[1];
        auto conv_ok = [](const Mod& c, long ci) { return c.ia[0] == ci && c.ia[1] == 16 && c.kW() == 3 && c.kH() == 3 && c.padW() == 1 && c.padH() == 1; };
        if (!conv_ok(*d.conv1, d.Cin) || !conv_ok(*d.conv2, 16)) return false;
        const long K3 = 16L * (d.S / 2) * (d.S / 2);
        if (M(L.kids[6]).ia[7] != 1 || M(L.kids[6]).ia[0] != K3 || d.lin1->ia[0] != K3 || d.lin1->ia[1] != 64 || d.lin2->ia[0] != 64) return false;
        d.slope = M(L.kids[2]).fa[0];
        if (M(L.kids[4]).fa[0] != d.slope || M(L.kids[8]).fa[0] != d.slope) return false;
        if (!(d.slope > 0.f)) return false;
        const Mod &am = M(q.kids[1]), &ag = M(q.kids[2]);
        d.ur = (int)am.ia[0]; d.us = (int)am.ia[1]; d.ut = (int)am.ia[2]; d.Hg = (int)ag.ia[0]; d.Wg = (int)ag.ia[1];
        if (d.P != d.ur + d.us + 2 * d.ut) return false;
        return cg_locnet_supported(d.S, d.Cin, d.P) != 0;
    }
    static void loc_weights(const vector<Mod*>& qs, Net* n, const float* w[48]) {
        for (size_t b = 0; b < qs.size(); ++b) {
            const Mod& L = *n->mods[qs[b]->kids[0]];
            const Mod *c1 = n->mods[L.kids[1]].get(), *c2 = n->mods[L.kids[3]].get(), *l1 = n->mods[L.kids[7]].get(), *l2 = n->mods[L.kids[9]].get();
            const float* v[12] = {c1->w, c1->b, c2->w, c2->b, l1->w, l1->b, l2->w, l2->b, c1->wf, c1->wb, c2->wf, c2->wb};
            for (int k = 0; k < 12; ++k) w[12 * b + k] = v[k];
        }
    }
    vector<Val> fwd_loc(const vector<Mod*>& qs, const Val& in, const LocDesc& d) {
        const KTable* k = K();
        const int G = (int)qs.size();
        Mod& q0 = *qs[0];
        const long N = in.d[0], S_ = d.S, Cin = d.Cin, K3 = 16L * (S_ / 2) * (S_ / 2);
        Val pooled = buf(q0, "loc.pooled", {G * N, Cin, S_, S_}, NHWC), h1 = buf(q0, "loc.h1", {G * N, 16, S_, S_}, NHWC),
            m2 = buf(q0, "loc.m2", {G * N, 16, S_, S_}, NHWC), h2 = buf(q0, "loc.h2", {G * N, K3}), h3 = buf(q0, "loc.h3", {G * N, 64}),
            prm = buf(q0, "loc.params", {G * N, d.P}), grid = buf(q0, "loc.grid", {G * N, d.Hg, d.Wg, 2});
        for (Mod* q : qs) {
            const Mod& L = M(q->kids[0]);
            need_plain(M(L.kids[1]), false); need_plain(M(L.kids[3]), false);
        }
        Net* n_ = net; vector<Mod*> qv = qs; const LocDesc dd = d; Val x = in;
        emit([=](Run& c) {
            const float* w[48];
            loc_weights(qv, n_, w);
            return k->locnet_forward(c.CS(), G, (int)N, c.P(x), 1, w, dd.S, dd.Cin, dd.P, dd.ur, dd.us, dd.ut, dd.slope, dd.Hg, dd.Wg, c.P(pooled), c.P(h1),
                                     c.P(m2), c.P(h2), c.P(h3), c.P(prm), c.P(grid));
        });
        vector<Val> outs = slices(grid, G);
        for (int b = 0; b < G; ++b) {
            MS& s = S(*qs[b]);
            s.out = outs[b]; s.loc_fused = true; s.locG = G; s.locN = N;
            s.ran_set = false;
        }
        MS& s0 = S(q0);
        s0.x = in;
        return outs;
    }
    vector<Val> bwd_loc(const vector<Mod*>& qs, const vector<Val>& gouts, bool acc) {
        const KTable* k = K();
        const int G = (int)qs.size();
        Mod& q0 = *qs[0];
        MS& s0 = S(q0);
        LocDesc d;
        if (!match_loc(q0, s0.x, d)) { err("cg_net: fused localisation branch lost its shape"); return gouts; }
        const long N = s0.locN, S_ = d.S, Cin = d.Cin, K3 = 16L * (S_ / 2) * (S_ / 2);
        Val GG = gather(q0, gouts, gouts[0]);
        Val pooled = buf(q0, "loc.pooled", {G * N, Cin, S_, S_}, NHWC), h1 = buf(q0, "loc.h1", {G * N, 16, S_, S_}, NHWC),
            m2 = buf(q0, "loc.m2", {G * N, 16, S_, S_}, NHWC), h2 = buf(q0, "loc.h2", {G * N, K3}), h3 = buf(q0, "loc.h3", {G * N, 64}),
            prm = buf(q0, "loc.params", {G * N, d.P});
        Val ga1 = buf(q0, "loc.ga1", {G * N, 16, S_, S_}, NHWC), ga2 = buf(q0, "loc.ga2", {G * N, 16, S_, S_}, NHWC), g3 = buf(q0, "loc.g3", {G * N, 64}),
            g4 = buf(q0, "loc.g4", {G * N, d.P}), gx = buf(q0, "loc.gx", {G * N, Cin, 2 * S_, 2 * S_}, NHWC);
        Net* n_ = net; vector<Mod*> qv = qs; const LocDesc dd = d;
        emit([=](Run& c) {
            const float* w[48];
            loc_weights(qv, n_, w);
            return k->locnet_backward(c.CS(), G, (int)N, w, dd.S, dd.Cin, dd.P, dd.ur, dd.us, dd.ut, dd.slope, dd.Hg, dd.Wg, c.P(h1), c.P(m2), c.P(h3), c.P(prm),
                                      c.P(GG), c.P(ga1), c.P(ga2), c.P(g3), c.P(g4), c.P(gx));
        });
        if (acc) {
            wg_fork();
            const long P_ = d.P;
            MS* s0p = &s0;
            wg_after_dgrad([this, G, N, S_, Cin, K3, P_, pooled, ga1, h1, ga2, h2, g3, h3, g4, qv, s0p]() {
            struct W { int li; Val x, dy; Geo g; };
            const W ws_[4] = {
                {1, pooled, ga1, Geo{(int)N, (int)S_, (int)S_, (int)Cin, 16, 3, 3, 1, 1, 0}},
                {3, h1, ga2, Geo{(int)N, (int)S_, (int)S_, 16, 16, 3, 3, 1, 1, 0}},
                {7, h2, g3, Geo{(int)N, 1, 1, (int)K3, 64, 1, 1, 0, 0, 0}},
                {9, h3, g4, Geo{(int)N, 1, 1, 64, (int)P_, 1, 1, 0, 0, 0}}};
            for (int wi = 0; wi < 4; ++wi) {
                const W& wv = ws_[wi];
                const size_t xs = (size_t)wv.x.phys() / G * 4, ds = (size_t)wv.dy.phys() / G * 4;
                vector<Mod*> lay; vector<PrepAcc> ap;
                for (int b = 0; b < G; ++b) {
                    lay.push_back(&M(M(qv[b]->kids[0]).kids[wv.li]));
                    ap.push_back(PrepAcc{wv.x.at(b * xs), wv.dy.at(b * ds), wv.g});
                }
                emit_wgrad_group(lay, ap, s0p->loc_ws[wi], s0p->loc_ws_bytes[wi]);
            }
            });
        }
        return share_gin(qs, gx);
    }

    std::string signature(const Mod& m) {
        std::string s = "(" + std::to_string(m.kind);
        for (int i = 0; i < 8; ++i) s += "," + std::to_string(m.ia[i]);
        char b[64]; snprintf(b, sizeof b, ",%a,%a,%d", m.fa[0], m.fa[1], m.train); s += b;
        for (int c : m.kids) s += signature(M(c));
        return s + ")";
    }
    vector<vector<int>> branch_groups(const Mod& q) {
        vector<std::pair<std::string, vector<int>>> by;
        for (size_t i = 0; i < q.kids.size(); ++i) {
            std::string sg = signature(M(q.kids[i]));
            bool found = false;
            for (auto& e : by) if (net->grouped && e.first == sg) { e.second.push_back((int)i); found = true; break; }
            if (!found) by.push_back({sg, {(int)i}});
        }
        vector<vector<int>> groups;
        for (auto& e : by)
            for (size_t k0 = 0; k0 < e.second.size(); k0 += 4) groups.emplace_back(e.second.begin() + k0, e.second.begin() + std::min(k0 + 4, e.second.size()));
        std::sort(groups.begin(), groups.end(), [](const vector<int>& a, const vector<int>& b) { return a[0] < b[0]; });
        return groups;
    }
    void run_groups(const vector<std::function<void()>>& thunks) {
        const bool multi = net->grouped && net->overlap_groups && thunks.size() > 1 && cs == 0 && thunks.size() <= 4;
        if (!multi) { for (auto& f : thunks) f(); return; }
        emit_event(EV_RECORD, EV_FORK, 0);
        for (size_t t = 1; t < thunks.size(); ++t) {
            const int sidx = (int)t;
            use_stream(sidx);
            cs = sidx;
            emit_event(EV_WAIT, EV_FORK, 0);
            thunks[t]();
            flush_wgrad();
            emit_event(EV_RECORD, EV_JOIN, sidx);
            cs = 0;
        }
        thunks[0]();
        for (size_t t = 1; t < thunks.size(); ++t) emit_event(EV_WAIT, EV_JOIN, (int)t);
    }
    enum { EV_RECORD = 0, EV_WAIT = 1 };
    enum { EV_FORK = 0, EV_JOIN, EV_WGFORK, EV_WGJOIN };
    void emit_event(int what, int kind, int k) {
        static const char* const names[] = {"fork", "join", "wgfork", "wgjoin"};
        const int s = cs;
        const std::string line = std::string(what == EV_RECORD ? "event|record|" : "event|wait|") + names[kind] + (kind == EV_FORK ? "" : std::to_string(k)) +
                                 "|s" + std::to_string(s);
        emit([=](Run& c) {
            Net* n = c.net;
            if (n->trace) { trace_note(n, line); return 0; }
            const hipEvent_t e = kind == EV_FORK ? n->fork_ev : kind == EV_JOIN ? n->side_ev[k - 1] : kind == EV_WGFORK ? n->wg_fork_ev[k] : n->wg_join_ev[k];
            const hipStream_t st = (hipStream_t)c.S(s);
            return (what == EV_RECORD ? hipEventRecord(e, st) : hipStreamWaitEvent(st, e, 0)) == hipSuccess ? 0 : 1;
        });
    }
    void flush_wgrad() {
        if (dry || !pend[cs]) return;
        const KTable* k = K();
        emit([=](Run& c) { return k->conv2d_wgrad_flush(c.CS()); });
        pend[cs] = 0;
    }
    bool wg_on() const { return net->wgrad_stream && net->fusion && acc_pass && !dry && cs < 4; }
    void wg_fork() {
        if (!wg_on()) return;
        emit_event(EV_RECORD, EV_WGFORK, cs);
    }
    int wg_enter() {
        const int s = cs;
        if (!wg_on()) return s;
        use_stream(4 + s);
        cs = 4 + s;
        emit_event(EV_WAIT, EV_WGFORK, s);
        wg_used[s] = true; wg_unjoined[s] = true;
        return s;
    }
    void wg_leave(int s) { cs = s; }
    void wg_before_dgrad() { wg_fork(); }
    void wg_after_dgrad(std::function<void()> f) {
        const int s_ = wg_enter(); f(); wg_leave(s_);
    }
    void wg_join_all() {
        if (dry) return;
        const int back = cs;
        for (int s = 0; s < 4; ++s) {
            if (!wg_used[s]) continue;
            cs = 4 + s;
            flush_wgrad();
            emit_event(EV_RECORD, EV_WGJOIN, s);
            cs = 0;
            emit_event(EV_WAIT, EV_WGJOIN, s);
            wg_used[s] = false;
        }
        cs = back;
    }
    long count_draws(Mod& m, const Val& in) {
        Prog tmp; tmp.net = net;
        Prog* save = pr;
        pr = &tmp; ++dry;
        GCtx ctx{{0}};
        gfwd({&m}, {in}, ctx);
        --dry; pr = save;
        return ctx.cur[0];
    }
    Val fwd_concat(Mod& q, const Val& in, Mod* drop = nullptr) {
        const KTable* k = K();
        const int nb = (int)q.kids.size();
        vector<Val> outs(nb);
        vector<long> base(nb);
        for (int i = 0; i < nb; ++i) { base[i] = rng; rng += count_draws(M(q.kids[i]), in); }
        vector<std::function<void()>> thunks;
        for (auto& idxs : branch_groups(q)) {
            thunks.push_back([&, idxs]() {
                GCtx ctx; vector<Mod*> mods; vector<Val> ins;
                for (int i : idxs) { ctx.cur.push_back(base[i]); mods.push_back(&M(q.kids[i])); ins.push_back(in); }
                vector<Val> res = gfwd(mods, ins, ctx);
                for (size_t t = 0; t < idxs.size(); ++t) outs[idxs[t]] = as_nhwc(res[t]);
            });
        }
        run_groups(thunks);
        const long N = outs[0].d[0], H = outs[0].d[2], W = outs[0].d[3];
        MS& s = S(q);
        s.sizes.clear();
        long Ct = 0; bool all4 = true;
        for (auto& o : outs) { s.sizes.push_back(o.d[1]); Ct += o.d[1]; all4 = all4 && o.d[1] % 4 == 0; }
        Val out = buf(q, "out", {N, Ct, H, W}, NHWC);
        s.cat_drop = false;
        if (drop && net->fusion && net->cat_fuse && nb <= 4 && all4) {
            vector<long> sz = s.sizes;
            MS& sd = S(*drop);
            Val noise = buf(*drop, "noise", {N, Ct});
            const long off = rng; rng += N * Ct;
            const float pdrop = drop->fa[0];
            emit([=](Run& c) {
                const float* src[4]; int cc[4];
                for (int i = 0; i < nb; ++i) { src[i] = c.P(outs[i]); cc[i] = (int)sz[i]; }
                return k->concat_channels_dropout(c.CS(), nb, src, cc, c.P(out), c.P(noise), (int)N, H * W, 1.0f - pdrop, 1.0f, c.seed, c.roff + (uint64_t)off, c.rbase);
            });
            s.cat_drop = true;
            s.out = Val();
            sd.noise = noise; sd.out = out;
            return out;
        }
        if (net->fusion && net->cat_fuse && nb <= 4 && all4) {
            vector<long> sz = s.sizes;
            emit([=](Run& c) {
                const float* src[4]; int cc[4];
                for (int i = 0; i < nb; ++i) { src[i] = c.P(outs[i]); cc[i] = (int)sz[i]; }
                return k->concat_channels(c.CS(), nb, src, cc, c.P(out), N * H * W);
            });
        } else {
            long off = 0;
            for (int i = 0; i < nb; ++i) {
                const long ci = s.sizes[i], o_ = off; Val src = outs[i];
                emit([=](Run& c) { return k->copy_channels(c.CS(), c.P(src), c.P(out), N * H * W, (int)ci, 0, (int)Ct, (int)o_, (int)ci); });
                off += ci;
            }
        }
        s.out = out;
        if (drop) return fwd(*drop, out);
        return out;
    }
    Val bwd_concat(Mod& q, const Val& in, const Val& go_, bool acc, Mod* drop = nullptr) {
        const KTable* k = K();
        const int nb = (int)q.kids.size();
        MS& s = S(q);
        const bool masked = drop && s.cat_drop;
        Val go = go_;
        if (drop && !masked) go = bwd(*drop, s.out, go_, acc);
        Val g = as_nhwc(go);
        const long N = g.d[0], Ct = g.d[1], H = g.d[2], W = g.d[3];
        vector<Val> dst(nb); vector<bool> have(nb, false);
        vector<vector<int>> groups = branch_groups(q);
        if (net->stacking) {
            for (auto& idxs : groups) {
                bool eq = idxs.size() > 1;
                for (int i : idxs) eq = eq && s.sizes[i] == s.sizes[idxs[0]];
                if (!eq) continue;
                Val block = buf(q, "gslice_block" + std::to_string(idxs[0]), {(long)idxs.size() * N, s.sizes[idxs[0]], H, W}, NHWC);
                vector<Val> sl = split(block, (int)idxs.size());
                for (size_t t = 0; t < idxs.size(); ++t) { dst[idxs[t]] = sl[t]; have[idxs[t]] = true; }
            }
        }
        bool all4 = true;
        for (int i = 0; i < nb; ++i) {
            if (!have[i]) dst[i] = buf(q, "gslice" + std::to_string(i), {N, s.sizes[i], H, W}, NHWC);
            all4 = all4 && s.sizes[i] % 4 == 0;
        }
        if (masked) {
            vector<long> sz = s.sizes;
            Val noise = S(*drop).noise;
            emit([=](Run& c) {
                float* d_[4]; int cc[4];
                for (int i = 0; i < nb; ++i) { d_[i] = c.P(dst[i]); cc[i] = (int)sz[i]; }
                return k->split_channels_masked(c.CS(), nb, c.P(g), c.P(noise), d_, cc, (int)N, H * W);
            });
            S(*drop).gin = Val();
        } else if (net->fusion && net->cat_fuse && nb <= 4 && all4) {
            vector<long> sz = s.sizes;
            emit([=](Run& c) {
                float* d_[4]; int cc[4];
                for (int i = 0; i < nb; ++i) { d_[i] = c.P(dst[i]); cc[i] = (int)sz[i]; }
                return k->split_channels(c.CS(), nb, c.P(g), d_, cc, N * H * W);
            });
        } else {
            long off = 0;
            for (int i = 0; i < nb; ++i) {
                const long ci = s.sizes[i], o_ = off; Val d_ = dst[i];
                emit([=](Run& c) { return k->copy_channels(c.CS(), c.P(g), c.P(d_), N * H * W, (int)Ct, (int)o_, (int)ci, 0, (int)ci); });
                off += ci;
            }
        }
        vector<Val> grads(nb);
        vector<std::function<void()>> thunks;
        for (auto& idxs : groups) {
            thunks.push_back([&, idxs]() {
                vector<Mod*> mods; vector<Val> ins, gs;
                for (int i : idxs) { mods.push_back(&M(q.kids[i])); ins.push_back(in); gs.push_back(dst[i]); }
                vector<Val> res = gbwd(mods, ins, gs, acc);
                for (size_t t = 0; t < idxs.size(); ++t) grads[idxs[t]] = as_nhwc(res[t]);
            });
        }
        run_groups(thunks);
        Val accv = buf_like(q, "gsum", grads[0], NHWC);
        const long n = accv.phys();
        if (net->fusion && net->cat_fuse && nb >= 2 && nb <= 4 && grads[0].phys() % 4 == 0) {
            emit([=](Run& c) {
                const float* src[4];
                for (int i = 0; i < nb; ++i) src[i] = c.P(grads[i]);
                return k->sum_n(c.CS(), nb, src, c.P(accv), n);
            });
        } else {
            Val g0 = grads[0];
// ... 587 lines not shown
```

### cat-generator_amd/csrc/runtime.hip

```cpp
#include "common.h"
#include <stdarg.h>
#include <stdlib.h>
#include <chrono>
#include <mutex>
#include <unordered_map>
#include <vector>

namespace cg {
char* err_buf() {
    static thread_local char buf[512] = {0};
    return buf;
}
int fail(const char* fmt, ...) {
    va_list ap;
    va_start(ap, fmt);
    vsnprintf(err_buf(), 512, fmt, ap);
    va_end(ap);
    return 1;
}

namespace {
struct OptDef { const char* name; long dflt; };
const OptDef kOptDefs[OPT_COUNT] = {
    {"CG_SKINNY", 1}, {"CG_GEMM_BK32", 1}, {"CG_WINO_BK", 0}, {"CG_NN_TILE", 0}, {"CG_TN_TILE", 0}, {"CG_NN_SPLITS", 0}, {"CG_TN_SPLITS", 0},
    {"CG_XCD_SWIZZLE", 7}, {"CG_NN_GLDS", 1}, {"CG_TN_GLDS", 1}, {"CG_WINO_GLDS", 1}, {"CG_PAD_SKIP", 20}, {"CG_WINO3", 1},
    {"CG_WINO_DGRAD_FUSE", 1}, {"CG_WINO_DGRAD_FUSE_LAUNCHES", 0}, {"CG_WINO3_LAUNCHES", 0}, {"CG_PACK_WIDE", 1},
    {"CG_SAMPLER_ATOMIC_LAUNCHES", 0},
};
long g_opt_val[OPT_COUNT];
int g_opt_state[OPT_COUNT];
}

void* col_scratch(hipStream_t stream) {
    constexpr int kPool = 8, kReserve = 4;
    static std::unordered_map<hipStream_t, void*> blocks;
    static std::vector<void*> pool;
    static std::mutex mu;
    std::lock_guard<std::mutex> lk(mu);
    auto it = blocks.find(stream);
    if (it != blocks.end()) return it->second;
    hipStreamCaptureStatus st = hipStreamCaptureStatusNone;
    const bool capturing = stream && hipStreamIsCapturing(stream, &st) == hipSuccess && st != hipStreamCaptureStatusNone;
    if (capturing && pool.empty()) {
        cg::fail("column reduce: no scratch block left for a stream first used inside a graph capture (run one pass on it before cg_graph_begin)");
        return nullptr;
    }
    if (!capturing && (int)pool.size() <= kReserve) {
        char* p = nullptr;
        hipStreamCaptureMode mode = hipStreamCaptureModeRelaxed;
        (void)hipThreadExchangeStreamCaptureMode(&mode);
        const bool ok = hipMalloc((void**)&p, kColScratchBytes * kPool) == hipSuccess &&
                        hipMemsetAsync(p, 0, kColScratchBytes * kPool, stream) == hipSuccess &&
                        hipStreamSynchronize(stream) == hipSuccess;
        (void)hipThreadExchangeStreamCaptureMode(&mode);
        if (!ok) {
            (void)hipGetLastError();
            if (pool.empty()) { cg::fail("column reduce: cannot allocate %zu bytes of scratch", kColScratchBytes * kPool); return nullptr; }
        } else
            for (int i = kPool - 1; i >= 0; --i) pool.insert(pool.begin(), p + (size_t)i * kColScratchBytes);
    }
    void* blk = pool.back();
    pool.pop_back();
    blocks[stream] = blk;
    return blk;
}
namespace {
__global__ void queue_probe_spin_k(unsigned long long ticks, int* sink) {
    const unsigned long long t0 = wall_clock64();
    while (wall_clock64() - t0 < ticks) { }
    if (ticks == ~0ull) *sink = 1;
}
struct QueuePool {
    std::vector<hipStream_t> s;
    std::unordered_map<hipStream_t, std::vector<int>> cls;
    std::mutex mu;
};
QueuePool& qpool() { static QueuePool p; return p; }
constexpr int kQueuePool = 24;

double probe_pair(hipStream_t a, hipStream_t b, bool both, unsigned long long ticks) {
    (void)hipStreamSynchronize(a);
    if (both) (void)hipStreamSynchronize(b);
    const auto t0 = std::chrono::steady_clock::now();
    hipLaunchKernelGGL(queue_probe_spin_k, dim3(1), dim3(64), 0, a, ticks, (int*)nullptr);
    if (both) hipLaunchKernelGGL(queue_probe_spin_k, dim3(1), dim3(64), 0, b, ticks, (int*)nullptr);
    (void)hipStreamSynchronize(a);
    if (both) (void)hipStreamSynchronize(b);
    return std::chrono::duration<double, std::milli>(std::chrono::steady_clock::now() - t0).count();
}
bool same_queue(hipStream_t a, hipStream_t b) {
    const unsigned long long ticks = 30000;
    int votes = 0;
    for (int r = 0; r < 3; ++r) {
        const double one = probe_pair(a, a, false, ticks), two = probe_pair(a, b, true, ticks);
        if (two > 1.6 * one) ++votes;
    }
    return votes >= 2;
}
}

int queue_classify(hipStream_t ref) {
    QueuePool& p = qpool();
    hipStreamCaptureStatus st = hipStreamCaptureStatusNone;
    if (ref && hipStreamIsCapturing(ref, &st) == hipSuccess && st != hipStreamCaptureStatusNone)
        return cg::fail("queue_stream: a stream's hardware queue cannot be probed inside a graph capture (run one pass on it before cg_graph_begin)");
    while ((int)p.s.size() < kQueuePool) {
        hipStream_t q;
        if (hipStreamCreateWithFlags(&q, hipStreamNonBlocking) != hipSuccess) return cg::fail("queue_stream: hipStreamCreate failed");
        p.s.push_back(q);
    }
    std::vector<int> c(p.s.size(), -1);
    std::vector<hipStream_t> rep;
    for (size_t i = 0; i < p.s.size(); ++i) {
        if (same_queue(ref, p.s[i])) { c[i] = 0; continue; }
        for (size_t k = 0; k < rep.size() && c[i] < 0; ++k)
            if (same_queue(rep[k], p.s[i])) c[i] = (int)k + 1;
        if (c[i] < 0) { rep.push_back(p.s[i]); c[i] = (int)rep.size(); }
    }
    (void)hipGetLastError();
    p.cls[ref] = c;
    return 0;
}

hipStream_t queue_stream(hipStream_t ref, int cls, int slot) {
    QueuePool& p = qpool();
    std::lock_guard<std::mutex> lk(p.mu);
    if (!p.cls.count(ref) && queue_classify(ref)) return nullptr;
    const std::vector<int>& c = p.cls[ref];
    int nclass = 0;
    for (int v : c) nclass = std::max(nclass, v + 1);
    if (nclass < 2) {
        static bool warned = false;
        if (!warned) { warned = true; fprintf(stderr, "cg: the hardware-queue probe found one queue only - side streams are plain pool streams (overlap not guaranteed)\n"); }
        return p.s[(size_t)((cls & 3) * (kQueuePool / 4) + slot % (kQueuePool / 4)) % p.s.size()];
    }
    cls = cls % nclass;
    int seen = 0;
    hipStream_t last = nullptr;
    for (size_t i = 0; i < c.size(); ++i)
        if (c[i] == cls) { last = p.s[i]; if (seen++ == slot) return p.s[i]; }
    if (last) return last;
    cg::fail("queue_stream: no pool stream on hardware queue class %d", cls);
    return nullptr;
}

int queue_class(hipStream_t ref, hipStream_t s) {
    if (s == ref) return 0;
    QueuePool& p = qpool();
    std::lock_guard<std::mutex> lk(p.mu);
    auto it = p.cls.find(ref);
    if (it == p.cls.end()) return -1;
    for (size_t i = 0; i < p.s.size(); ++i) if (p.s[i] == s) return it->second[i];
    return -1;
}

unsigned long g_opt_epoch = 1;
long opt(Opt o) {
    if (g_opt_state[o] == 0) {
        const char* e = getenv(kOptDefs[o].name);
        g_opt_val[o] = e ? atol(e) : kOptDefs[o].dflt;
        g_opt_state[o] = 1;
    }
    return g_opt_val[o];
}
void opt_count(Opt o) { opt(o); ++g_opt_val[o]; }
}

extern "C" {

int cg_abi_version(void) { return CG_TIMING_PROBE ? -1 : CG_ABI_VERSION; }
int cg_set_option(const char* name, long value) {
    CG_REQUIRE(name, "cg_set_option: null name");
    for (int i = 0; i < cg::OPT_COUNT; ++i)
        if (strcmp(name, cg::kOptDefs[i].name) == 0) {
            ++cg::g_opt_epoch;
            if (value == -1) { cg::g_opt_state[i] = 0; return 0; }
            cg::g_opt_val[i] = value; cg::g_opt_state[i] = 2;
            return 0;
        }
    return cg::fail("cg_set_option: unknown option %s", name);
}
int cg_get_option(const char* name, long* value) {
    CG_REQUIRE(name && value, "cg_get_option: null pointer");
    for (int i = 0; i < cg::OPT_COUNT; ++i)
        if (strcmp(name, cg::kOptDefs[i].name) == 0) { *value = cg::opt((cg::Opt)i); return 0; }
    return cg::fail("cg_get_option: unknown option %s", name);
}
const char* cg_last_error(void) { return cg::err_buf(); }
int cg_device_count(int* count) { CG_REQUIRE(count, "null"); CG_HIP(hipGetDeviceCount(count)); return 0; }
int cg_set_device(int device) { CG_HIP(hipSetDevice(device)); return 0; }
int cg_malloc(void** dptr, size_t bytes) { CG_REQUIRE(dptr, "null"); CG_HIP(hipMalloc(dptr, bytes)); return 0; }
int cg_free(void* dptr) { CG_HIP(hipFree(dptr)); return 0; }
int cg_memcpy_h2d(void* stream, void* dst, const void* src, size_t bytes) {
    CG_HIP(hipMemcpyAsync(dst, src, bytes, hipMemcpyHostToDevice, cg::S(stream))); return 0;
}
int cg_memcpy_d2h(void* stream, void* dst, const void* src, size_t bytes) {
    CG_HIP(hipMemcpyAsync(dst, src, bytes, hipMemcpyDeviceToHost, cg::S(stream)));
    CG_HIP(hipStreamSynchronize(cg::S(stream)));
    return 0;
}
int cg_memcpy_d2d(void* stream, void* dst, const void* src, size_t bytes) {
    CG_HIP(hipMemcpyAsync(dst, src, bytes, hipMemcpyDeviceToDevice, cg::S(stream))); return 0;
}
__global__ __launch_bounds__(256) void zero16_k(float4* __restrict__ p, long n16) {
    const float4 z = make_float4(0.f, 0.f, 0.f, 0.f);
    CG_GRID_STRIDE(i, n16) p[i] = z;
}
int cg_memset_zero(void* stream, void* dst, size_t bytes) {
    if (bytes >= (1u << 20) && (uintptr_t)dst % 16 == 0) {
        const long n16 = (long)(bytes / 16);
        CG_EW_LAUNCH(zero16_k, n16, (float4*)dst, n16);
        const size_t done = (size_t)n16 * 16;
        if (done < bytes) CG_HIP(hipMemsetAsync((char*)dst + done, 0, bytes - done, cg::S(stream)));
        return 0;
    }
    CG_HIP(hipMemsetAsync(dst, 0, bytes, cg::S(stream))); return 0;
}
int cg_stream_create(void** stream) {
    CG_REQUIRE(stream, "null");
    hipStream_t s; CG_HIP(hipStreamCreateWithFlags(&s, hipStreamNonBlocking)); *stream = (void*)s; return 0;
}
int cg_stream_on_queue(void* ref_stream, int queue_class, int slot, void** stream) {
    CG_REQUIRE(stream && queue_class >= 0 && slot >= 0, "cg_stream_on_queue: bad arguments");
    hipStream_t s = cg::queue_stream(cg::S(ref_stream), queue_class, slot);
    if (!s) return 1;
    *stream = (void*)s;
    return 0;
}
int cg_stream_destroy(void* stream) { CG_HIP(hipStreamDestroy(cg::S(stream))); return 0; }
int cg_stream_sync(void* stream) { CG_HIP(hipStreamSynchronize(cg::S(stream))); return 0; }

int cg_host_alloc(void** hptr, size_t bytes) {
    CG_REQUIRE(hptr && bytes > 0, "cg_host_alloc: bad arguments");
    CG_HIP(hipHostMalloc(hptr, bytes, hipHostMallocDefault));
    return 0;
}
int cg_host_free(void* hptr) { if (hptr) CG_HIP(hipHostFree(hptr)); return 0; }
int cg_event_create(void** event) {
    CG_REQUIRE(event, "cg_event_create: null pointer");
    hipEvent_t e; CG_HIP(hipEventCreateWithFlags(&e, hipEventDisableTiming)); *event = (void*)e; return 0;
}
int cg_event_destroy(void* event) { if (event) CG_HIP(hipEventDestroy((hipEvent_t)event)); return 0; }
int cg_event_record(void* event, void* stream) {
    CG_REQUIRE(event, "cg_event_record: null event");
    CG_HIP(hipEventRecord((hipEvent_t)event, cg::S(stream))); return 0;
}
int cg_event_sync(void* event) {
    CG_REQUIRE(event, "cg_event_sync: null event");
    CG_HIP(hipEventSynchronize((hipEvent_t)event)); return 0;
}
int cg_stream_wait_event(void* stream, void* event) {
    CG_REQUIRE(event, "cg_stream_wait_event: null event");
    CG_HIP(hipStreamWaitEvent(cg::S(stream), (hipEvent_t)event, 0)); return 0;
}
}
```

### cat-generator_amd/csrc/wgrad_finish.hip

```cpp
#include "common.h"
#include <mutex>
#include <unordered_map>
#include <vector>

namespace {

using cg::f4c;
using cg::ld4;
using cg::phase_map;
using cg::sel4;

template <bool UPS, int STEP>
__device__ __forceinline__ float fold(const float* pg, int tap, int ci, int co, int Cin, int Cout, int k, int pad, int kp, long plane, int S,
                                      long sstride, int sp0) {
    float s = 0.f;
    if (UPS) {
        const int dy = tap / k, dx = tap - dy * k;
        for (int sp = sp0; sp < S; sp += STEP)
#pragma unroll
            for (int p = 0; p < 4; ++p) {
                const int tp = phase_map(p >> 1, dy, pad) * kp + phase_map(p & 1, dx, pad);
                s += pg[(long)sp * sstride + (long)p * plane + ((long)tp * Cin + ci) * Cout + co];
            }
    } else {
        const long o = ((long)tap * Cin + ci) * Cout + co;
        constexpr int kInFlight = STEP == 8 ? 4 : 1;
#pragma unroll kInFlight
        for (int sp = sp0; sp < S; sp += STEP) s += pg[(long)sp * sstride + o];
    }
    return s;
}

__device__ __forceinline__ void add4(float4& s, const float4& p) { s.x += p.x; s.y += p.y; s.z += p.z; s.w += p.w; }
template <int STEP>
__device__ __forceinline__ float4 fold4(const float* src, int S, long sstride, int sp0) {
    float4 s = make_float4(0.f, 0.f, 0.f, 0.f);
    int sp = sp0;
    for (; sp + 3 * STEP < S; sp += 4 * STEP) {
        const float4 p0 = ld4(src + (long)sp * sstride), p1 = ld4(src + (long)(sp + STEP) * sstride);
        const float4 p2 = ld4(src + (long)(sp + 2 * STEP) * sstride), p3 = ld4(src + (long)(sp + 3 * STEP) * sstride);
        add4(s, p0); add4(s, p1); add4(s, p2); add4(s, p3);
    }
    for (; sp < S; sp += STEP) add4(s, ld4(src + (long)sp * sstride));
    return s;
}

__device__ __forceinline__ float lane_groups_sum(float (*sh)[33], int ol) {
    float t = 0.f;
#pragma unroll
    for (int r = 0; r < 8; ++r) t += sh[r][ol];
    return t;
}

__device__ __forceinline__ void bias_sum_block(float (*sh)[33], const float* bp, float* gb, int c0, int S, int P, long bsstride, int Cout, float scale) {
    const int cl = threadIdx.x & 31, ln = threadIdx.x >> 5;
    const int c = c0 + cl;
    float s = 0.f;
    if (c < Cout)
        for (int i = ln; i < S * P; i += 8) s += bp[(long)(i / P) * bsstride + (long)(i % P) * Cout + c];
    sh[ln][cl] = s;
    __syncthreads();
    if (ln == 0 && c < Cout) gb[c] += scale * lane_groups_sum(sh, cl);
}

template <bool UPS>
__global__ __launch_bounds__(256) void wgrad_reduce_kernel(const float* part, float* gw, int Cin, int Cout, int k, int KK,
                                                           int pad, int kp, int S, float scale, int CI_T, long sstride) {
    extern __shared__ float sh[];
    const int ci0 = blockIdx.x * CI_T, co0 = blockIdx.y * 32;
    const long plane = (long)(UPS ? kp * kp : KK) * Cin * Cout;
    const int n1 = KK * CI_T * 32;
    for (int idx = threadIdx.x; idx < n1; idx += 256) {
        const int co_l = idx & 31;
        const int r = idx >> 5;
        const int ci_l = r % CI_T, tap = r / CI_T;
        const int ci = ci0 + ci_l, co = co0 + co_l;
        float s = 0.f;
        if (ci < Cin && co < Cout) s = fold<UPS, 1>(part, tap, ci, co, Cin, Cout, k, pad, kp, plane, S, sstride, 0);
        sh[(ci_l * KK + tap) * 33 + co_l] = s;
    }
    __syncthreads();
    const int run = CI_T * KK;
    for (int idx = threadIdx.x; idx < n1; idx += 256) {
        const int j = idx % run, co_l = idx / run;
        const int ci_l = j / KK, tap = j - ci_l * KK;
        const int ci = ci0 + ci_l, co = co0 + co_l;
        if (ci < Cin && co < Cout) {
            float* dst = gw + ((long)co * Cin + ci) * KK + tap;
            *dst += scale * sh[j * 33 + co_l];
        }
    }
}

__global__ __launch_bounds__(256) void bias_part_reduce_kernel(const float* bp, float* gb, int S, int P, long sstride, int Cout, float scale) {
    __shared__ float sh[8][33];
    bias_sum_block(sh, bp, gb, blockIdx.x * 32, S, P, sstride, Cout, scale);
}

struct RedPtrs { float* gw0; float* gw1; float* gw2; float* gw3; float* gb0; float* gb1; float* gb2; float* gb3;
                 long gws; };
struct RedJob {
    const float* part; const float* bias_part;
    RedPtrs rp;
    long sstride, gstride, bsstride;
    int Cin, Cout, k, KK, pad, kp, S, P, ups, ngroups, wblocks, bblocks;
    int block0;
    float scale;
    int tr;
    int v4;
};
constexpr int kRedJobs = 20;
struct RedJobTable { RedJob j[kRedJobs]; int n; };

__device__ __forceinline__ float* gw_of(const RedPtrs& rp, int group) {
    return rp.gws ? rp.gw0 + (long)group * rp.gws : sel4(group, rp.gw0, rp.gw1, rp.gw2, rp.gw3);
}

template <bool UPS>
__device__ __forceinline__ void wgrad_reduce_small(float (*sh)[33], const RedJob& J, int group, int bx) {
    const int ol = threadIdx.x & 31, ln = threadIdx.x >> 5;
    const long total = (long)J.KK * J.Cin * J.Cout, plane = (long)(UPS ? J.kp * J.kp : J.KK) * J.Cin * J.Cout;
    const long i = bx * 32L + ol;
    int co = 0, ci = 0, tap = 0;
    float s = 0.f;
    if (i < total) {
        co = (int)(i % J.Cout);
        const long r = i / J.Cout;
        ci = (int)(r % J.Cin);
        tap = (int)(r / J.Cin);
        s = fold<UPS, 8>(J.part + (long)group * J.gstride, tap, ci, co, J.Cin, J.Cout, J.k, J.pad, J.kp, plane, J.S, J.sstride, ln);
    }
    sh[ln][ol] = s;
    __syncthreads();
    if (ln == 0 && i < total) gw_of(J.rp, group)[((long)co * J.Cin + ci) * J.KK + tap] += J.scale * lane_groups_sum(sh, ol);
}

__device__ __forceinline__ void wgrad_reduce_small_v4(float* shf, const RedJob& J, int group, int bx) {
    float4* sh4 = reinterpret_cast<float4*>(shf);
    const int ol = threadIdx.x & 31, ln = threadIdx.x >> 5;
    const long total = (long)J.KK * J.Cin * J.Cout;
    const long i = bx * 128L + 4 * ol;
    float4 s = make_float4(0.f, 0.f, 0.f, 0.f);
    if (i < total) s = fold4<8>(J.part + (long)group * J.gstride + i, J.S, J.sstride, ln);
    sh4[ln * 32 + ol] = s;
    __syncthreads();
    if (ln < 4 && i < total) {
        float t = 0.f;
#pragma unroll
        for (int r = 0; r < 8; ++r) t += f4c(sh4[r * 32 + ol], ln);
        const long e = i + ln;
        const int co = (int)(e % J.Cout);
        const long rr = e / J.Cout;
        const int ci = (int)(rr % J.Cin), tap = (int)(rr / J.Cin);
        gw_of(J.rp, group)[((long)co * J.Cin + ci) * J.KK + tap] += J.scale * t;
    }
}

__device__ __forceinline__ void wgrad_reduce_t_tile(float (*t)[33], const float* __restrict__ pg, float* __restrict__ gw, int ci0, int co0,
                                                    int Cin, int Cout, int S, long sstride, float scale) {
    const int tx = threadIdx.x & 31, ty = threadIdx.x >> 5;
    if ((Cout & 3) == 0 && (sstride & 3) == 0 && ((uintptr_t)pg & 15) == 0) {
        const int r = threadIdx.x >> 3, c4 = threadIdx.x & 7;
        const float4 s = fold4<1>(pg + (long)(ci0 + r) * Cout + co0 + 4 * c4, S, sstride, 0);
        t[r][4 * c4] = s.x; t[r][4 * c4 + 1] = s.y; t[r][4 * c4 + 2] = s.z; t[r][4 * c4 + 3] = s.w;
    } else
#pragma unroll
    for (int r = ty; r < 32; r += 8) t[r][tx] = fold<false, 1>(pg, 0, ci0 + r, co0 + tx, Cin, Cout, 1, 0, 0, 0, S, sstride, 0);
    __syncthreads();
#pragma unroll
    for (int r = ty; r < 32; r += 8) gw[(long)(co0 + r) * Cin + ci0 + tx] += scale * t[tx][r];
}
__global__ __launch_bounds__(256) void wgrad_reduce_t_kernel(const float* __restrict__ part, float* __restrict__ gw0, long gws, int Cin,
                                                             int Cout, int S, long sstride, long gstride, float scale) {
    __shared__ float t[32][33];
    const int group = blockIdx.z;
    wgrad_reduce_t_tile(t, part + (long)group * gstride, gw0 + (long)group * gws, blockIdx.x * 32, blockIdx.y * 32, Cin, Cout, S, sstride, scale);
}

__device__ __forceinline__ void red_block(float (*sh)[33], const RedJob& J, int group, int bx) {
    if (bx >= J.wblocks) {
        float* gb = sel4(group, J.rp.gb0, J.rp.gb1, J.rp.gb2, J.rp.gb3);
        if (gb) bias_sum_block(sh, J.bias_part + (long)group * J.P * J.Cout, gb, (bx - J.wblocks) * 32, J.S, J.P, J.bsstride, J.Cout, J.scale);
    } else if (J.tr) {
        const int nci = J.Cin / 32;
        wgrad_reduce_t_tile(sh, J.part + (long)group * J.gstride, gw_of(J.rp, group), (bx % nci) * 32, (bx / nci) * 32, J.Cin, J.Cout, J.S, J.sstride, J.scale);
    } else if (J.v4)
        wgrad_reduce_small_v4(&sh[0][0], J, group, bx);
    else if (J.ups)
        wgrad_reduce_small<true>(sh, J, group, bx);
    else
        wgrad_reduce_small<false>(sh, J, group, bx);
}

__global__ __launch_bounds__(256) void wgrad_reduce_small_kernel(RedJob J) {
    __shared__ __attribute__((aligned(16))) float sh[32][33];
    red_block(sh, J, (int)blockIdx.y, (int)blockIdx.x);
}

__global__ __launch_bounds__(256) void wgrad_reduce_batch_kernel(RedJobTable t) {
    __shared__ __attribute__((aligned(16))) float sh[32][33];
    const int b = (int)blockIdx.x;
    int ji = 0;
    for (int q = 1; q < t.n; ++q)
        if (b >= t.j[q].block0) ji = q;
    const RedJob& J = t.j[ji];
    const int per = J.wblocks + J.bblocks;
    const int group = (b - J.block0) / per;
    red_block(sh, J, group, (b - J.block0) - group * per);
}

std::mutex g_red_mu;
std::unordered_map<hipStream_t, std::vector<RedJob>> g_red_queue;

bool transposable(const cg::WgradParts& w) { return w.kH * w.kW == 1 && !w.ups && w.Cin % 32 == 0 && w.Cout % 32 == 0; }

RedJob red_job(const cg::WgradParts& w, bool defer) {
    RedJob job;
    memset(&job, 0, sizeof(job));
    const int nptr = w.gws ? 1 : w.ngroups;
    cg::set4(job.rp.gw0, job.rp.gw1, job.rp.gw2, job.rp.gw3, w.gw, nptr);
    cg::set4(job.rp.gb0, job.rp.gb1, job.rp.gb2, job.rp.gb3, w.gb, nptr);
    job.rp.gws = w.gws;
    job.part = w.part; job.bias_part = w.bias_part;
    job.Cin = w.Cin; job.Cout = w.Cout; job.k = w.kH; job.KK = w.kH * w.kW; job.pad = w.pad; job.ups = w.ups ? 1 : 0;
    job.kp = w.ups ? cg::phase_kp(w.kH, w.pad) : 0;
    job.S = w.S; job.P = w.ups ? 4 : 1; job.ngroups = w.ngroups; job.scale = w.scale;
    const long relems = (long)job.KK * w.Cin * w.Cout;
    job.gstride = (w.ups ? 4L * job.kp * job.kp : job.KK) * w.Cin * w.Cout;
    job.sstride = w.ngroups * job.gstride;
    job.bsstride = (long)w.ngroups * job.P * w.Cout;
    job.wblocks = cg::cdiv(relems, 32); job.bblocks = w.bias_part ? cg::cdiv(w.Cout, 32) : 0;
    if (defer && transposable(w)) {
        job.tr = 1; job.wblocks = (w.Cin / 32) * (w.Cout / 32);
    } else if (!w.ups && w.Cout % 4 == 0 && cg::al16(w.part) && job.sstride % 4 == 0 && job.gstride % 4 == 0) {
        job.v4 = 1; job.wblocks = cg::cdiv(relems, 128);
    }
    return job;
}

int small_reduce(hipStream_t st, bool defer, const RedJob& job) {
    if (defer) {
        std::lock_guard<std::mutex> lk(g_red_mu);
        g_red_queue[st].push_back(job);
        return 0;
    }
    hipLaunchKernelGGL(wgrad_reduce_small_kernel, dim3(job.wblocks + job.bblocks, job.ngroups), dim3(256), 0, st, job);
    CG_LAUNCH_CHECK();
    return 0;
}

}

int cg::wgrad_finish(hipStream_t st, const WgradParts& w, bool defer) {
    const RedJob job = red_job(w, defer);
    const int Cin = w.Cin, Cout = w.Cout, KK = job.KK;
    if (w.gws && transposable(w) && !w.bias_part) {
        hipLaunchKernelGGL(wgrad_reduce_t_kernel, dim3(Cin / 32, Cout / 32, w.ngroups), dim3(256), 0, st, w.part, w.gw[0], w.gws, Cin, Cout, w.S,
                           job.sstride, job.gstride, w.scale);
        CG_LAUNCH_CHECK();
        return 0;
    }
    int ci_t = KK == 1 ? 64 : 8;
    while (ci_t > 1 && (size_t)KK * ci_t * 33 * sizeof(float) > 60000) ci_t >>= 1;
    const size_t shb = (size_t)KK * ci_t * 33 * sizeof(float);
    const dim3 rgrid(cg::cdiv(Cin, ci_t), cg::cdiv(Cout, 32));
    if ((long)rgrid.x * rgrid.y < cg::kNumCU) return small_reduce(st, defer, job);
    for (int gi = 0; gi < w.ngroups; ++gi) {
        const float* pg = w.part + gi * job.gstride;
        float* gwi = w.gws ? w.gw[0] + gi * w.gws : w.gw[gi];
        hipLaunchKernelGGL(w.ups ? wgrad_reduce_kernel<true> : wgrad_reduce_kernel<false>, rgrid, dim3(256), shb, st, pg, gwi, Cin, Cout, w.kH, KK,
                           w.pad, job.kp, w.S, w.scale, ci_t, job.sstride);
        CG_LAUNCH_CHECK();
        if (w.gb && w.gb[gi]) {
            hipLaunchKernelGGL(bias_part_reduce_kernel, dim3(cg::cdiv(Cout, 32)), dim3(256), 0, st, w.bias_part + (long)gi * job.P * Cout, w.gb[gi],
                               w.S, job.P, job.bsstride, Cout, w.scale);
            CG_LAUNCH_CHECK();
        }
    }
    return 0;
}

void cg::wgrad_discard_all() {
    std::lock_guard<std::mutex> lk(g_red_mu);
    for (auto& kv : g_red_queue) kv.second.clear();
}

extern "C" {

int cg_conv2d_wgrad_pending(void* stream, int* njobs) {
    CG_REQUIRE(njobs, "cg_conv2d_wgrad_pending: null pointer");
    std::lock_guard<std::mutex> lk(g_red_mu);
    auto it = g_red_queue.find(cg::S(stream));
    *njobs = it == g_red_queue.end() ? 0 : (int)it->second.size();
    return 0;
}

int cg_conv2d_wgrad_flush(void* stream) {
    hipStream_t st = cg::S(stream);
    std::vector<RedJob> jobs;
    {
        std::lock_guard<std::mutex> lk(g_red_mu);
        auto it = g_red_queue.find(st);
        if (it == g_red_queue.end() || it->second.empty()) return 0;
        jobs.swap(it->second);
    }
    for (size_t j0 = 0; j0 < jobs.size(); j0 += kRedJobs) {
        RedJobTable t;
        memset(&t, 0, sizeof(t));
        t.n = (int)std::min<size_t>(kRedJobs, jobs.size() - j0);
        int blocks = 0;
        for (int q = 0; q < t.n; ++q) {
            t.j[q] = jobs[j0 + q];
            t.j[q].block0 = blocks;
            blocks += t.j[q].ngroups * (t.j[q].wblocks + t.j[q].bblocks);
        }
        hipLaunchKernelGGL(wgrad_reduce_batch_kernel, dim3(blocks), dim3(256), 0, st, t);
        CG_LAUNCH_CHECK();
    }
    return 0;
}

}
```

### include/catgan.h

```cpp
#ifndef CATGAN_H
#define CATGAN_H

#include <stddef.h>
#include <stdint.h>

#ifdef __cplusplus
extern "C" {
#endif

#define CG_ABI_VERSION 2

int         cg_abi_version(void);
const char* cg_last_error(void);
int cg_set_option(const char* name, long value);
int cg_get_option(const char* name, long* value);
int cg_device_count(int* count);
int cg_set_device(int device);
int cg_malloc(void** dptr, size_t bytes);
int cg_free(void* dptr);
int cg_memcpy_h2d(void* stream, void* dst, const void* src, size_t bytes);
int cg_memcpy_d2h(void* stream, void* dst, const void* src, size_t bytes);
int cg_memcpy_d2d(void* stream, void* dst, const void* src, size_t bytes);
int cg_memset_zero(void* stream, void* dst, size_t bytes);
int cg_stream_create(void** stream);
int cg_stream_on_queue(void* ref_stream, int queue_class, int slot, void** stream);
int cg_stream_destroy(void* stream);
int cg_stream_sync(void* stream);
int cg_host_alloc(void** hptr, size_t bytes);
int cg_host_free(void* hptr);
int cg_event_create(void** event);
int cg_event_destroy(void* event);
int cg_event_record(void* event, void* stream);
int cg_event_sync(void* event);
int cg_stream_wait_event(void* stream, void* event);
int cg_images_u8_to_f32(void* stream, const unsigned char* src, float* dst, long npixels, int colorspace);
int cg_images_u8_scale_to_f32(void* stream, const unsigned char* src, float* dst, int N, int Hs, int Ws, int Hd, int Wd, int colorspace);
int cg_images_u8_augment_to_f32(void* stream, const unsigned char* src, float* dst, int N, int Hs, int Ws, int Hd, int Wd,
                                int colorspace, const float* desc, float noise_std, uint64_t seed, uint64_t offset);
int cg_images_u8_gather_scale_to_f32(void* stream, const unsigned char* set, long M, const int32_t* idx, float* dst, int N, int Hs, int Ws,
                                     int Hd, int Wd, int colorspace);
int cg_images_u8_gather_augment_to_f32(void* stream, const unsigned char* set, long M, const int32_t* idx, float* dst, int N, int Hs, int Ws,
                                       int Hd, int Wd, int colorspace, const float* desc, float noise_std, uint64_t seed, uint64_t offset);
int cg_images_u8_augment_window_to_f32(void* stream, const unsigned char* src, float* dst, int N, int Hp, int Wp, int margin, int Hd, int Wd,
                                       int colorspace, const float* desc, float noise_std, uint64_t seed, uint64_t offset);
int cg_images_u8_gather_augment_window_to_f32(void* stream, const unsigned char* set, long M, const int32_t* idx, float* dst, int N, int Hp,
                                              int Wp, int margin, int Hd, int Wd, int colorspace, const float* desc, float noise_std,
                                              uint64_t seed, uint64_t offset);
int cg_faces_u8_extract(void* stream, const unsigned char* src, size_t src_bytes, const uint64_t* src_off, const int32_t* geom,
                        const float* inv, const int32_t* taps, size_t ntaps, const uint64_t* tap_off, unsigned char* dst, int N, int out,
                        void* workspace, size_t workspace_bytes);
int cg_faces_u8_extract_variants(void* stream, const unsigned char* src, size_t src_bytes, const uint64_t* src_off, const int32_t* geom,
                                 const float* inv, const int32_t* taps, size_t ntaps, const uint64_t* tap_off, int pad, int A,
                                 const float* desc, const uint64_t* bases, float noise_scale, uint64_t seed, unsigned char* dst, int N, int out,
                                 void* workspace, size_t workspace_bytes);
int cg_faces_u8_extract_padded(void* stream, const unsigned char* src, size_t src_bytes, const uint64_t* src_off, const int32_t* geom,
                               const float* inv, const int32_t* taps, size_t ntaps, const uint64_t* tap_off, const int32_t* pads,
                               unsigned char* dst, int N, int out, void* workspace, size_t workspace_bytes);
int cg_colorspace_convert(void* stream, const float* src, float* dst, long npixels, int from, int to);
size_t cg_nearest_workspace_bytes(int N, int Q, long D);
int cg_nearest_update(void* stream, const float* pool, int N, long D, const float* queries, int Q, int index0, int reset, float* best_d2,
                      int32_t* best_idx, void* workspace);

size_t cg_conv2d_workspace_bytes(int N, int Hp, int Wp, int Cin, int Cout,
                                 int kH, int kW, int padH, int padW, int ups);
int cg_conv2d_forward(void* stream, const float* x, const float* wpk, const float* bias,
                      float* y, int N, int Hp, int Wp, int Cin, int Cout,
                      int kH, int kW, int padH, int padW, int ups,
                      void* ws, size_t ws_bytes);

size_t cg_conv2d_workspace_bytes_grouped(int ngroups, int N, int Hp, int Wp, int Cin, int Cout,
                                         int kH, int kW, int padH, int padW, int ups);
int cg_conv2d_forward_grouped(void* stream, int ngroups, const float* const* x, const float* const* wpk,
                              const float* const* bias, float* const* y, int N, int Hp, int Wp, int Cin, int Cout,
                              int kH, int kW, int padH, int padW, int ups, void* ws, size_t ws_bytes);

size_t cg_conv2d_stats_rows(int N, int Hp, int Wp, int Cin, int Cout, int kH, int kW, int padH, int padW, int ups);
int cg_conv2d_forward_ex(void* stream, int ngroups, const float* const* x, const float* const* wpk,
                         const float* const* bias, float* const* y, int N, int Hp, int Wp, int Cin, int Cout,
                         int kH, int kW, int padH, int padW, int ups,
                         int act, float slope, const float* const* alpha, float* const* y_act, float* stats,
                         void* ws, size_t ws_bytes);

size_t cg_conv2d_dgrad_ups2_workspace_bytes(int N, int Hp, int Wp, int Cin, int Cout, int k, int pad);
int cg_conv2d_dgrad_ups2(void* stream, const float* dy, const float* wb_ph, float* dx_lo,
                         int N, int Hp, int Wp, int Cin, int Cout, int k, int pad,
                         void* ws, size_t ws_bytes);

size_t cg_conv2d_wgrad_workspace_bytes(int N, int Hp, int Wp, int Cin, int Cout,
                                       int kH, int kW, int padH, int padW, int ups);
int cg_conv2d_wgrad(void* stream, const float* x, const float* dy, float* gw_canonical, float* gb,
                    int N, int Hp, int Wp, int Cin, int Cout,
                    int kH, int kW, int padH, int padW, int ups, float scale,
                    void* ws, size_t ws_bytes);

size_t cg_conv2d_wgrad_workspace_bytes_grouped(int ngroups, int N, int Hp, int Wp, int Cin, int Cout,
                                               int kH, int kW, int padH, int padW, int ups);
int cg_conv2d_wgrad_grouped(void* stream, int ngroups, const float* const* x, const float* const* dy,
                            float* const* gw_canonical, float* const* gb, int N, int Hp, int Wp, int Cin, int Cout,
                            int kH, int kW, int padH, int padW, int ups, float scale, void* ws, size_t ws_bytes);
int cg_conv2d_wgrad_grouped_deferred(void* stream, int ngroups, const float* const* x, const float* const* dy,
                            float* const* gw_canonical, float* const* gb, int N, int Hp, int Wp, int Cin, int Cout,
                            int kH, int kW, int padH, int padW, int ups, float scale, void* ws, size_t ws_bytes);
int cg_conv2d_wgrad_flush(void* stream);
int cg_conv2d_wgrad_gemm(void* stream, const float* x, const float* dy, int N, int Hp, int Wp, int Cin, int Cout,
                         int kH, int kW, int padH, int padW, int ups, void* ws, size_t ws_bytes);
int cg_conv2d_wgrad_pending(void* stream, int* njobs);
size_t cg_conv2d_wgrad_workspace_bytes_strided(int ngroups, int N, int Hp, int Wp, int Cin, int Cout,
                                               int kH, int kW, int padH, int padW, int ups);
int cg_conv2d_wgrad_strided(void* stream, int ngroups, const float* x, long x_stride, const float* dy, long dy_stride,
                            float* gw_canonical, long gw_stride, int N, int Hp, int Wp, int Cin, int Cout,
                            int kH, int kW, int padH, int padW, int ups, float scale, void* ws, size_t ws_bytes);

int cg_bias_grad(void* stream, const float* dy, float* gb, long M, int C, float scale,
                 void* ws, size_t ws_bytes);

size_t cg_pack_conv_weight_floats(int Cout, int Cin, int kH, int kW);
int cg_pack_conv_weight(void* stream, const float* w_canonical, float* wf, float* wb,
                        int Cout, int Cin, int kH, int kW);
int cg_pack_conv_weight_batch(void* stream, int n, const float* const* w_canonical, float* const* wf, float* const* wb,
                              const int* Cout, const int* Cin, const int* kH, const int* kW, const int* wb_map);
int cg_pack_conv_weight_map(void* stream, const float* w_canonical, float* wf, float* wbT, int Cout, int Cin, int kH, int kW);
size_t cg_pack_conv_weight_ups2_floats(int Cout, int Cin, int k, int pad);
int cg_pack_conv_weight_ups2(void* stream, const float* w_canonical, float* wf_ph, float* wb_ph,
                             int Cout, int Cin, int k, int pad);

size_t cg_conv2d_ups2_wino_supported(int N, int Hp, int Wp, int Cin, int Cout, int k, int pad);
size_t cg_conv2d_ups2_wino_v_floats(int N, int Hp, int Wp, int C);
size_t cg_conv2d_ups2_wino_u_floats(int Cin, int Cout);
int cg_conv2d_ups2_wino_pack(void* stream, const float* wf_ph, const float* wb_ph, float* u_fwd, float* u_bwd,
                             int Cout, int Cin);
int cg_conv2d_ups2_wino_gemm(void* stream, const float* v, const float* u, const float* bias, float* y,
                             int N, int Hp, int Wp, int Cin, int Cout, int dgrad);
int cg_conv2d_ups2_wino_forward(void* stream, const float* x_lo, const float* u_fwd, const float* bias, float* y,
                                float* v, int N, int Hp, int Wp, int Cin, int Cout);
size_t cg_conv2d_ups2_wino_stats_rows(int N, int Hp, int Wp, int Cin, int Cout);
int cg_conv2d_ups2_wino_forward_stats(void* stream, const float* x_lo, const float* u_fwd, const float* bias, float* y,
                                      float* v, int N, int Hp, int Wp, int Cin, int Cout, float* stats);
size_t cg_conv2d_ups2_wino22_supported(int N, int Hp, int Wp, int Cin, int Cout);
size_t cg_conv2d_ups2_wino22_dgrad_supported(int N, int Hp, int Wp, int Cin, int Cout);
size_t cg_conv2d_ups2_wino22_v_floats(int N, int Hp, int Wp, int Cin);
size_t cg_conv2d_ups2_wino22_u_floats(int Cin, int Cout);
int cg_conv2d_ups2_wino22_pack(void* stream, const float* wf_ph, const float* wb_ph, float* u_fwd, float* u_bwd, int Cout, int Cin);
int cg_conv2d_ups2_wino22_forward_stats(void* stream, const float* x_lo, const float* u22, const float* bias, float* y,
                                        float* v, int N, int Hp, int Wp, int Cin, int Cout, float* stats);
size_t cg_conv2d_ups2_wino22_dgrad_v_floats(int N, int Hp, int Wp, int Cin, int Cout);
int cg_conv2d_ups2_wino22_dgrad(void* stream, const float* dy, const float* u_bwd, float* dx_lo, float* v_dy,
                                int N, int Hp, int Wp, int Cin, int Cout);
int cg_conv2d_ups2_wino_dgrad(void* stream, const float* dy, const float* u_bwd, float* dx_lo, float* v_dy,
                              int N, int Hp, int Wp, int Cin, int Cout);
size_t cg_conv2d_ups2_wino_dgrad_part_floats(int N, int Hp, int Wp, int Cin, int Cout);
int cg_conv2d_ups2_wino_dgrad_split(void* stream, const float* dy, const float* u_bwd, float* dx_lo, float* v_dy, float* part,
                                    int N, int Hp, int Wp, int Cin, int Cout);
size_t cg_conv2d_ups2_wino_wgrad_workspace_bytes(int N, int Hp, int Wp, int Cin, int Cout);
int cg_conv2d_ups2_wino_wgrad(void* stream, const float* v, const float* dy, float* gw_canonical, float* gb,
                              int N, int Hp, int Wp, int Cin, int Cout, float scale, void* ws, size_t ws_bytes);

int cg_prelu_forward(void* stream, const float* x, const float* alpha, float* y, long n);
size_t cg_prelu_backward_workspace_bytes(long n);
int cg_prelu_backward(void* stream, const float* x, const float* dy, const float* alpha,
                      float* dx, float* galpha, float scale, long n, void* ws, size_t ws_bytes);
size_t cg_prelu_backward_grouped_workspace_bytes(int ngroups, long n_per_group);
int cg_prelu_backward_grouped(void* stream, const float* x, const float* dy, const float* const* alpha, float* dx,
                              float* const* galpha, float scale, int ngroups, long n_per_group, void* ws, size_t ws_bytes);
int cg_leakyrelu_forward(void* stream, const float* x, float* y, float slope, long n);
int cg_leakyrelu_backward(void* stream, const float* x, const float* dy, float* dx, float slope, long n);
int cg_sigmoid_forward(void* stream, const float* x, float* y, long n);
int cg_sigmoid_backward(void* stream, const float* y, const float* dy, float* dx, long n);

int cg_bce_forward(void* stream, const float* p, const float* t, float* loss, long n);
int cg_bce_backward(void* stream, const float* p, const float* t, float* dp, long n);

int cg_mse_forward(void* stream, const float* x, const float* t, float* loss, long n);
int cg_mse_backward(void* stream, const float* x, const float* t, float* dx, long n);

int cg_bn_stats(void* stream, const float* x, long M, int C, double* sums);
int cg_bn_forward(void* stream, const float* x, float* y, const float* gamma, const float* beta,
                  const double* sums, double count, long M, int C, float eps, float momentum,
                  float* running_mean, float* running_var, float* save_mean, float* save_invstd);
int cg_bn_backward_stats(void* stream, const float* x, const float* dy, const float* save_mean,
                         const float* save_invstd, long M, int C, double* sums);
int cg_bn_backward(void* stream, const float* x, const float* dy, const float* gamma,
                   const float* save_mean, const float* save_invstd,
                   const double* sums, double count, const double* local_sums,
                   long M, int C, float* dx, float* ggamma, float* gbeta, float scale);
int cg_bn_forward_eval(void* stream, const float* x, float* y, const float* gamma, const float* beta,
                       const float* running_mean, const float* running_var, long M, int C, float eps);

int cg_bn_stats_finalize(void* stream, const float* partials, long rows, int C, double* sums);
int cg_bn_running_update(void* stream, const double* sums, double count, int C, float momentum, float* running_mean, float* running_var);
int cg_bn_act_forward(void* stream, const float* x, float* y, const float* gamma, const float* beta,
                      const double* sums, double count, long M, int C, float eps, float momentum,
                      float* running_mean, float* running_var, float* save_mean, float* save_invstd, const float* alpha);
size_t cg_bn_act_backward_sums(int C);
int cg_bn_act_backward_stats(void* stream, const float* x, const float* dy, const float* save_mean,
                             const float* save_invstd, const float* gamma, const float* beta, const float* alpha,
                             long M, int C, double* sums);
int cg_bn_act_backward(void* stream, const float* x, const float* dy, const float* gamma, const float* beta,
                       const float* save_mean, const float* save_invstd, const float* alpha,
                       const double* sums, double count, const double* local_sums, long M, int C,
                       float* dx, float* ggamma, float* gbeta, float* galpha, float scale);
int cg_act_pool2_mask_forward(void* stream, const float* x, float* y, const float* mask, int ngroups, int n_per_group,
                              int H, int W, int C, int act, float slope, const float* const* alpha, int pool_max);
size_t cg_act_pool2_mask_backward_workspace_bytes(int ngroups, int n_per_group, int H, int W, int C);
int cg_act_pool2_mask_backward(void* stream, const float* x, const float* gy, const float* mask, float* dx,
                               int ngroups, int n_per_group, int H, int W, int C, int act, float slope,
                               const float* const* alpha, float* const* galpha, float scale, int pool_max,
                               void* ws, size_t ws_bytes);

int cg_upsample2x_forward(void* stream, const float* x, float* y, int N, int H, int W, int C);
int cg_upsample2x_backward(void* stream, const float* dy, float* dx, int N, int H, int W, int C);
int cg_avgpool2_forward(void* stream, const float* x, float* y, int N, int H, int W, int C);
int cg_avgpool2_backward(void* stream, const float* dy, float* dx, int N, int H, int W, int C);
int cg_maxpool2_forward(void* stream, const float* x, float* y, int N, int H, int W, int C);
int cg_maxpool2_backward(void* stream, const float* x, const float* dy, float* dx, int N, int H, int W, int C);

int cg_mask_mul(void* stream, const float* x, const float* mask, float* y,
                int N, long HW, int C, int spatial);
int cg_rng_bernoulli(void* stream, float* out, long n, float keep_prob, float value,
                     uint64_t seed, uint64_t offset);
int cg_rng_uniform(void* stream, float* out, long n, float lo, float hi,
                   uint64_t seed, uint64_t offset);
int cg_rng_randint(void* stream, int32_t* out, long n, int32_t range, uint64_t seed, uint64_t offset);
int cg_rng_bernoulli_dev(void* stream, float* out, long n, float keep_prob, float value,
                         uint64_t seed, uint64_t offset, const uint64_t* base);
int cg_rng_uniform_dev(void* stream, float* out, long n, float lo, float hi,
                       uint64_t seed, uint64_t offset, const uint64_t* base);
int cg_rng_randint_dev(void* stream, int32_t* out, long n, int32_t range, uint64_t seed, uint64_t offset,
                       const uint64_t* base);
int cg_rng_bernoulli_dev_grouped(void* stream, float* out, long n_per_group, int ngroups, float keep_prob, float value,
                                 uint64_t seed, uint64_t off0, uint64_t off1, uint64_t off2, uint64_t off3,
                                 const uint64_t* base);
int cg_counter_add(void* stream, uint64_t* counter, uint64_t delta);

int cg_nchw_to_nhwc(void* stream, const float* in, float* out, int N, int C, int H, int W);
int cg_nhwc_to_nchw(void* stream, const float* in, float* out, int N, int C, int H, int W);
int cg_copy_channels(void* stream, const float* src, float* dst, long M,
                     int Csrc, int src_off, int Cdst, int dst_off, int Ccopy);
int cg_concat_channels(void* stream, int n, const float* const* src, const int* C, float* dst, long M);
int cg_split_channels(void* stream, int n, const float* src, float* const* dst, const int* C, long M);
int cg_sum_n(void* stream, int n, const float* const* src, float* out, long count);
int cg_concat_channels_dropout(void* stream, int n, const float* const* src, const int* C, float* dst, float* noise, int N, long HW,
                               float keep_prob, float value, uint64_t seed, uint64_t offset, const uint64_t* base);
int cg_split_channels_masked(void* stream, int n, const float* src, const float* noise, float* const* dst, const int* C, int N, long HW);
int cg_drop_linear_sigmoid_supported(int N, int F, int O);
int cg_drop_linear_sigmoid_forward(void* stream, const float* x, const float* w, const float* b, float* noise, float* xd, float* z, float* p,
                                   int N, int F, int O, float keep_prob, float value, uint64_t seed, uint64_t offset, const uint64_t* base);
int cg_drop_linear_sigmoid_backward(void* stream, const float* dp, const float* p, const float* xd, const float* noise, const float* w,
                                    float* gx, float* gw, float* gb, int N, int F, int O, float scale);
int cg_gather_rows(void* stream, const float* src, const int32_t* idx, float* dst,
                   long nrows, long rowlen);
int cg_fill(void* stream, float* x, float value, long n);
int cg_add(void* stream, const float* a, const float* b, float* out, long n);
int cg_axpy(void* stream, float alpha, const float* x, float* y, long n);
int cg_axpy_sign(void* stream, float alpha, const float* x, float* y, long n);
int cg_scale(void* stream, float* x, float alpha, long n);
int cg_clamp(void* stream, float* x, float lo, float hi, long n);
// ... 111 lines not shown
```

Baseline: 23450.

## Batch tail wgrad reductions into deferred launches and split final wgrad across streams

```diff
diff --git a/cat-generator_amd/csrc/common.h b/cat-generator_amd/csrc/common.h
--- a/cat-generator_amd/csrc/common.h
+++ b/cat-generator_amd/csrc/common.h
@@ -45,9 +45,10 @@
 enum Opt {
     OPT_SKINNY, OPT_GEMM_BK32, OPT_WINO_BK, OPT_NN_TILE, OPT_TN_TILE, OPT_NN_SPLITS, OPT_TN_SPLITS,
     OPT_XCD_SWIZZLE, OPT_NN_GLDS, OPT_TN_GLDS, OPT_WINO_GLDS, OPT_PAD_SKIP, OPT_WINO3, OPT_WINO_DGRAD_FUSE, OPT_WINO_DGRAD_FUSE_LAUNCHES,
-    OPT_WINO3_LAUNCHES, OPT_PACK_WIDE, OPT_SAMPLER_ATOMIC_LAUNCHES, OPT_COUNT
+    OPT_WINO3_LAUNCHES, OPT_PACK_WIDE, OPT_SAMPLER_ATOMIC_LAUNCHES, OPT_WGRAD_TAIL, OPT_COUNT
 };
 long opt(Opt o);
+bool opt_chosen(Opt o);
 void opt_count(Opt o);
 
 static inline int cdiv(long a, long b) { return (int)((a + b - 1) / b); }
@@ -80,7 +81,9 @@
     int ngroups, S, Cin, Cout, kH, kW, pad, ups;
     float scale;
 };
-int wgrad_finish(hipStream_t st, const WgradParts& w, bool defer);
+int wgrad_finish(hipStream_t st, const WgradParts& w, int defer);
+bool wgrad_finish_tiled(int Cin, int Cout, int KK);
+bool conv2d_wgrad_finish_tiled(int ngroups, int N, int Hp, int Wp, int Cin, int Cout, int kH, int kW, int padH, int padW, int ups);
 void wgrad_discard_all();
 
 constexpr int kSkinnyWgradBlocks = 512;
diff --git a/cat-generator_amd/csrc/gemm.hip b/cat-generator_amd/csrc/gemm.hip
--- a/cat-generator_amd/csrc/gemm.hip
+++ b/cat-generator_amd/csrc/gemm.hip
@@ -1462,19 +1462,24 @@
 namespace {
 int wgrad_impl(void* stream, int ngroups, const float* const* x, const float* const* dy, float* const* gw, float* const* gb, int N,
                int Hp, int Wp, int Cin, int Cout, int kH, int kW, int padH, int padW, int ups, float scale, void* ws, size_t ws_bytes,
-               bool defer, long xgs = 0, long dgs = 0, long gws = 0, bool gemm_only = false);
+               int defer, long xgs = 0, long dgs = 0, long gws = 0, bool gemm_only = false);
 }
 
 int cg_conv2d_wgrad_grouped(void* stream, int ngroups, const float* const* x, const float* const* dy, float* const* gw,
                             float* const* gb, int N, int Hp, int Wp, int Cin, int Cout, int kH, int kW, int padH, int padW,
                             int ups, float scale, void* ws, size_t ws_bytes) {
-    return wgrad_impl(stream, ngroups, x, dy, gw, gb, N, Hp, Wp, Cin, Cout, kH, kW, padH, padW, ups, scale, ws, ws_bytes, false);
+    return wgrad_impl(stream, ngroups, x, dy, gw, gb, N, Hp, Wp, Cin, Cout, kH, kW, padH, padW, ups, scale, ws, ws_bytes, 0);
 }
 
 int cg_conv2d_wgrad_grouped_deferred(void* stream, int ngroups, const float* const* x, const float* const* dy, float* const* gw,
                                      float* const* gb, int N, int Hp, int Wp, int Cin, int Cout, int kH, int kW, int padH, int padW,
                                      int ups, float scale, void* ws, size_t ws_bytes) {
-    return wgrad_impl(stream, ngroups, x, dy, gw, gb, N, Hp, Wp, Cin, Cout, kH, kW, padH, padW, ups, scale, ws, ws_bytes, true);
+    return wgrad_impl(stream, ngroups, x, dy, gw, gb, N, Hp, Wp, Cin, Cout, kH, kW, padH, padW, ups, scale, ws, ws_bytes, 1);
+}
+int cg_conv2d_wgrad_grouped_tail(void* stream, int ngroups, const float* const* x, const float* const* dy, float* const* gw,
+                                 float* const* gb, int N, int Hp, int Wp, int Cin, int Cout, int kH, int kW, int padH, int padW,
+                                 int ups, float scale, void* ws, size_t ws_bytes) {
+    return wgrad_impl(stream, ngroups, x, dy, gw, gb, N, Hp, Wp, Cin, Cout, kH, kW, padH, padW, ups, scale, ws, ws_bytes, 2);
 }
 
 int cg_conv2d_wgrad_strided(void* stream, int ngroups, const float* x, long x_stride, const float* dy, long dy_stride, float* gw,
@@ -1482,7 +1487,7 @@
                             float scale, void* ws, size_t ws_bytes) {
     CG_REQUIRE(x && dy && gw && x_stride > 0 && dy_stride > 0 && gw_stride > 0, "cg_conv2d_wgrad_strided: bad arguments");
     CG_REQUIRE(ngroups >= 1 && ngroups <= kMaxStridedGroups, "cg_conv2d_wgrad_strided: 1..%d groups per launch", kMaxStridedGroups);
-    return wgrad_impl(stream, ngroups, &x, &dy, &gw, nullptr, N, Hp, Wp, Cin, Cout, kH, kW, padH, padW, ups, scale, ws, ws_bytes, false,
+    return wgrad_impl(stream, ngroups, &x, &dy, &gw, nullptr, N, Hp, Wp, Cin, Cout, kH, kW, padH, padW, ups, scale, ws, ws_bytes, 0,
                       x_stride, dy_stride, gw_stride);
 }
 
@@ -1491,9 +1496,19 @@
     CG_REQUIRE(x && dy && ws, "cg_conv2d_wgrad_gemm: null pointer");
     CG_REQUIRE(!cg::skinny_ok(1, Cin, Cout, kH, kW, padH, padW, ups), "cg_conv2d_wgrad_gemm: this geometry runs the skinny kernel, not the GEMM");
     float* gw = (float*)ws;
-    return wgrad_impl(stream, 1, &x, &dy, &gw, nullptr, N, Hp, Wp, Cin, Cout, kH, kW, padH, padW, ups, 1.f, ws, ws_bytes, false, 0, 0, 0, true);
-}
-
+    return wgrad_impl(stream, 1, &x, &dy, &gw, nullptr, N, Hp, Wp, Cin, Cout, kH, kW, padH, padW, ups, 1.f, ws, ws_bytes, 0, 0, 0, 0, true);
+}
+
+namespace {
+bool head_wgrad_geom(int ngroups, int N, int Hp, int Wp, int Cin, int Cout, int kH, int kW, int padH, int padW, int ups) {
+    return ngroups == 1 && !ups && kH == Hp && kW == Wp && padH == 0 && padW == 0 && cg::opt(cg::OPT_PAD_SKIP) > 0 && cg::opt(cg::OPT_TN_GLDS) &&
+           cg::head_wgrad_ok(N, kH * kW, Cin, Cout);
+}
+}
+extern "C++" bool cg::conv2d_wgrad_finish_tiled(int ngroups, int N, int Hp, int Wp, int Cin, int Cout, int kH, int kW, int padH, int padW, int ups) {
+    if (!cg::skinny_ok(ngroups, Cin, Cout, kH, kW, padH, padW, ups) && head_wgrad_geom(ngroups, N, Hp, Wp, Cin, Cout, kH, kW, padH, padW, ups)) return false;
+    return cg::wgrad_finish_tiled(Cin, Cout, kH * kW);
+}
 namespace {
 void launch_tn_tile(const TNArgs& a, const TileCfg& tc, bool tng, dim3 grid, hipStream_t st, bool veca, bool vecb) {
     with_block_tile(tc, [&](auto t) {
@@ -1505,7 +1520,7 @@
 
 int wgrad_impl(void* stream, int ngroups, const float* const* x, const float* const* dy, float* const* gw, float* const* gb, int N,
                int Hp, int Wp, int Cin, int Cout, int kH, int kW, int padH, int padW, int ups, float scale, void* ws, size_t ws_bytes,
-               bool defer, long xgs, long dgs, long gws_, bool gemm_only) {
+               int defer, long xgs, long dgs, long gws_, bool gemm_only) {
     CG_REQUIRE(x && dy && gw, "cg_conv2d_wgrad: null pointer");
     const bool strided = xgs != 0;
     CG_REQUIRE(ngroups >= 1 && ngroups <= (strided ? kMaxStridedGroups : MAXG), "cg_conv2d_wgrad: 1..%d groups per launch", strided ? kMaxStridedGroups : MAXG);
@@ -1532,8 +1547,7 @@
         const cg::WgradParts parts{part, gb0 ? bpart : nullptr, gw, gb, 0, 1, blocks, Cin, Cout, 3, 3, 1, 0, scale};
         return cg::wgrad_finish(st, parts, defer);
     }
-    if (!strided && !gemm_only && ngroups == 1 && !ups && kH == Hp && kW == Wp && padH == 0 && padW == 0 && cg::opt(cg::OPT_PAD_SKIP) > 0 &&
-        cg::opt(cg::OPT_TN_GLDS) && cg::head_wgrad_ok(N, kH * kW, Cin, Cout) && x[0] && dy[0] && gw[0] && (uintptr_t)x[0] % 16 == 0 &&
+    if (!strided && !gemm_only && head_wgrad_geom(ngroups, N, Hp, Wp, Cin, Cout, kH, kW, padH, padW, ups) && x[0] && dy[0] && gw[0] && (uintptr_t)x[0] % 16 == 0 &&
         (uintptr_t)dy[0] % 16 == 0 && (uintptr_t)gw[0] % 4 == 0)
         return cg::head_wgrad(cg::S(stream), x[0], dy[0], gw[0], gb ? gb[0] : nullptr, N, kH * kW, Cin, Cout, scale) != 0;
     TNPlan p = plan_tn(g, ngroups);
diff --git a/cat-generator_amd/csrc/net.hip b/cat-generator_amd/csrc/net.hip
--- a/cat-generator_amd/csrc/net.hip
+++ b/cat-generator_amd/csrc/net.hip
@@ -227,7 +227,7 @@
     Val go = pr->out; go.ext = EXT_GY; go.off = 0; go.p = nullptr; go.fmt = gy_fmt; go.blk = 0; go.gi = go.gc = 0;
     Val gi = C.gbwd({&root}, {pr->in}, {go}, acc != 0, true)[0];
     if (C.failed) return cg::fail("%s", n->err);
-    if (acc) { C.buckets_start(); C.flush_wgrad(); C.wg_join_all(); }
+    if (acc) { C.buckets_start(); C.flush_wgrad(); C.wgrad_tail(); C.wg_join_all(); }
     CG_REQUIRE(!gi.is_tab, "cg_net_backward: the root module's gradInput is a table");
     pr->gin[acc] = gi;
     pr->have_bwd[acc] = true;
diff --git a/cat-generator_amd/csrc/net_compiler.h b/cat-generator_amd/csrc/net_compiler.h
--- a/cat-generator_amd/csrc/net_compiler.h
+++ b/cat-generator_amd/csrc/net_compiler.h
@@ -28,6 +28,11 @@
     bool wg_used[4] = {false, false, false, false};
     bool wg_unjoined[4] = {false, false, false, false};
     bool acc_pass = false;
+    struct WgRec { int sidx; size_t op; bool tiled; std::shared_ptr<int> mode; };
+    struct WgEnter { int sidx; size_t op; bool last; };
+    vector<WgRec> wg_recs;
+    vector<WgEnter> wg_enters;
+    int in_groups = 0;
 
     Compiler(Net* n, Prog* p) : net(n), pr(p) {}
     const KTable* K() const { return net->K; }
@@ -106,7 +111,13 @@
     template <class F> void emit(F f) {
         if (dry) return;
         ops->push_back(Op{cs, std::function<int(Run&)>(f)});
-    }
+        if (pre_next) { prepend(ops->size() - 1, pre_next); pre_next = nullptr; }
+    }
+    void prepend(size_t i, std::function<int(Run&)> pre) {
+        std::function<int(Run&)> fn = (*ops)[i].fn;
+        (*ops)[i].fn = [pre, fn](Run& c) { if (int rc = pre(c)) return rc; return fn(c); };
+    }
+    std::function<int(Run&)> pre_next;
     void use_stream(int sidx) { if (!dry && sidx + 1 > pr->nstreams) pr->nstreams = sidx + 1; }
 
     Val materialise(const Val& x) {
@@ -393,9 +404,15 @@
             if (!dry) pend[cs]++;
         } else ws_need(need);
         void* wsp = ws; const size_t wsb = ws_bytes;
+        std::shared_ptr<int> mode;
+        if (defer && !dry) {
+            mode = std::make_shared<int>(1);
+            wg_recs.push_back(WgRec{cs, ops->size(), cg::conv2d_wgrad_finish_tiled(G, GEO(g)), mode});
+        }
         emit([=](Run& c) {
             const float *x[4], *d_[4]; float *gw[4], *gb[4];
             for (int b = 0; b < G; ++b) { x[b] = c.P(ap[b].x); d_[b] = c.P(ap[b].dy); gw[b] = mods[b]->gw; gb[b] = mods[b]->gb; }
+            if (defer && *mode == 2) return k->conv2d_wgrad_grouped_tail(c.CS(), G, x, d_, gw, gb, GEO(g), c.scale, wsp, wsb);
             if (defer) return k->conv2d_wgrad_grouped_deferred(c.CS(), G, x, d_, gw, gb, GEO(g), c.scale, wsp, wsb);
             return k->conv2d_wgrad_grouped(c.CS(), G, x, d_, gw, gb, GEO(g), c.scale, c.W(), c.WB());
         });
@@ -1017,14 +1034,13 @@
             wg_fork();
             const long P_ = d.P;
             MS* s0p = &s0;
-            wg_after_dgrad([this, G, N, S_, Cin, K3, P_, pooled, ga1, h1, ga2, h2, g3, h3, g4, qv, s0p]() {
-            struct W { int li; Val x, dy; Geo g; };
-            const W ws_[4] = {
-                {1, pooled, ga1, Geo{(int)N, (int)S_, (int)S_, (int)Cin, 16, 3, 3, 1, 1, 0}},
-                {3, h1, ga2, Geo{(int)N, (int)S_, (int)S_, 16, 16, 3, 3, 1, 1, 0}},
-                {7, h2, g3, Geo{(int)N, 1, 1, (int)K3, 64, 1, 1, 0, 0, 0}},
-                {9, h3, g4, Geo{(int)N, 1, 1, 64, (int)P_, 1, 1, 0, 0, 0}}};
-            for (int wi = 0; wi < 4; ++wi) {
+            auto one = [this, G, N, S_, Cin, K3, P_, pooled, ga1, h1, ga2, h2, g3, h3, g4, qv, s0p](int wi) {
+                struct W { int li; Val x, dy; Geo g; };
+                const W ws_[4] = {
+                    {1, pooled, ga1, Geo{(int)N, (int)S_, (int)S_, (int)Cin, 16, 3, 3, 1, 1, 0}},
+                    {3, h1, ga2, Geo{(int)N, (int)S_, (int)S_, 16, 16, 3, 3, 1, 1, 0}},
+                    {7, h2, g3, Geo{(int)N, 1, 1, (int)K3, 64, 1, 1, 0, 0, 0}},
+                    {9, h3, g4, Geo{(int)N, 1, 1, 64, (int)P_, 1, 1, 0, 0, 0}}};
                 const W& wv = ws_[wi];
                 const size_t xs = (size_t)wv.x.phys() / G * 4, ds = (size_t)wv.dy.phys() / G * 4;
                 vector<Mod*> lay; vector<PrepAcc> ap;
@@ -1033,8 +1049,25 @@
                     ap.push_back(PrepAcc{wv.x.at(b * xs), wv.dy.at(b * ds), wv.g});
                 }
                 emit_wgrad_group(lay, ap, s0p->loc_ws[wi], s0p->loc_ws_bytes[wi]);
-            }
-            });
+            };
+            const bool last = wg_on() && cs == 0 && !in_groups;
+            int other = -1;
+            if (last && (wgrad_tail_bits() & 2))
+                for (int o = 3; o >= 1; --o) if (wg_used[o]) other = o;
+            if (!last) wg_after_dgrad([&]() { for (int wi = 0; wi < 4; ++wi) one(wi); });
+            else if (other < 0) {
+                const int s_ = wg_enter_beside(cs, true);
+                for (int wi = 0; wi < 4; ++wi) one(wi);
+                wg_leave(s_);
+            } else {
+                const int s_ = wg_enter_beside(cs, true);
+                one(0);
+                cs = s_; wg_enter_beside(other, true);
+                one(1);
+                cs = 4 + s_; one(2);
+                cs = 4 + other; one(3);
+                wg_leave(s_);
+            }
         }
         return share_gin(qs, gx);
     }
@@ -1062,6 +1095,7 @@
     }
     void run_groups(const vector<std::function<void()>>& thunks) {
         const bool multi = net->grouped && net->overlap_groups && thunks.size() > 1 && cs == 0 && thunks.size() <= 4;
+        struct Depth { int& d; explicit Depth(int& d_) : d(d_) { ++d; } ~Depth() { --d; } } depth(in_groups);
         if (!multi) { for (auto& f : thunks) f(); return; }
         emit_event(EV_RECORD, EV_FORK, 0);
         for (size_t t = 1; t < thunks.size(); ++t) {
@@ -1079,18 +1113,19 @@
     }
     enum { EV_RECORD = 0, EV_WAIT = 1 };
     enum { EV_FORK = 0, EV_JOIN, EV_WGFORK, EV_WGJOIN };
-    void emit_event(int what, int kind, int k) {
+    void emit_event(int what, int kind, int k) { emit(event_op(what, kind, k)); }
+    std::function<int(Run&)> event_op(int what, int kind, int k) {
         static const char* const names[] = {"fork", "join", "wgfork", "wgjoin"};
         const int s = cs;
         const std::string line = std::string(what == EV_RECORD ? "event|record|" : "event|wait|") + names[kind] + (kind == EV_FORK ? "" : std::to_string(k)) +
                                  "|s" + std::to_string(s);
-        emit([=](Run& c) {
+        return [=](Run& c) {
             Net* n = c.net;
             if (n->trace) { trace_note(n, line); return 0; }
             const hipEvent_t e = kind == EV_FORK ? n->fork_ev : kind == EV_JOIN ? n->side_ev[k - 1] : kind == EV_WGFORK ? n->wg_fork_ev[k] : n->wg_join_ev[k];
             const hipStream_t st = (hipStream_t)c.S(s);
             return (what == EV_RECORD ? hipEventRecord(e, st) : hipStreamWaitEvent(st, e, 0)) == hipSuccess ? 0 : 1;
-        });
+        };
     }
     void flush_wgrad() {
         if (dry || !pend[cs]) return;
@@ -1104,18 +1139,52 @@
         emit_event(EV_RECORD, EV_WGFORK, cs);
     }
     int wg_enter() {
+        return wg_on() ? wg_enter_beside(cs) : cs;
+    }
+    int wg_enter_beside(int o, bool last = false) {
         const int s = cs;
-        if (!wg_on()) return s;
-        use_stream(4 + s);
-        cs = 4 + s;
-        emit_event(EV_WAIT, EV_WGFORK, s);
-        wg_used[s] = true; wg_unjoined[s] = true;
+        use_stream(4 + o);
+        cs = 4 + o;
+        wg_enters.push_back(WgEnter{cs, ops->size(), last});
+        if (o == s) emit_event(EV_WAIT, EV_WGFORK, s);
+        else pre_next = event_op(EV_WAIT, EV_WGFORK, s);
+        wg_used[o] = true; wg_unjoined[o] = true;
         return s;
     }
     void wg_leave(int s) { cs = s; }
     void wg_before_dgrad() { wg_fork(); }
     void wg_after_dgrad(std::function<void()> f) {
         const int s_ = wg_enter(); f(); wg_leave(s_);
+    }
+    int wgrad_tail_bits() const {
+        if (!(acc_pass && net->wgrad_stream && defer_wg()) || net->world > 1) return 0;
+        if (net->trace && !cg::opt_chosen(cg::OPT_WGRAD_TAIL)) return 0;
+        return (int)cg::opt(cg::OPT_WGRAD_TAIL);
+    }
+    static constexpr int kTailWindow = 3;
+    void wgrad_tail() {
+        if (dry || !(wgrad_tail_bits() & 1)) return;
+        const KTable* k = K();
+        for (int s = 4; s < 8; ++s) {
+            vector<const WgRec*> r;
+            for (const WgRec& w : wg_recs) if (w.sidx == s) r.push_back(&w);
+            if (r.empty()) continue;
+            int t0 = -1;
+            for (int i = std::max(0, (int)r.size() - kTailWindow); i + 1 < (int)r.size(); ++i) if (r[i]->tiled) t0 = i;
+            if (t0 < 0 && r.back()->tiled) t0 = (int)r.size() - 1;
+            if (t0 >= 0) {
+                for (size_t i = (size_t)t0; i < r.size(); ++i) *r[i]->mode = 2;
+                continue;
+            }
+            const WgEnter* e = nullptr;
+            for (const WgEnter& w : wg_enters) if (w.sidx == s && w.last) e = &w;
+            if (!e) continue;
+            int queued = 0, before = 0;
+            for (const WgRec* w : r) if (w->op < e->op) { ++before; queued += !w->tiled; }
+            if (!queued) continue;
+            prepend(e->op, [=](Run& c) { return k->conv2d_wgrad_flush(c.CS()); });
+            pend[s] -= before;
+        }
     }
     void wg_join_all() {
         if (dry) return;
diff --git a/cat-generator_amd/csrc/runtime.hip b/cat-generator_amd/csrc/runtime.hip
--- a/cat-generator_amd/csrc/runtime.hip
+++ b/cat-generator_amd/csrc/runtime.hip
@@ -25,7 +25,7 @@
     {"CG_SKINNY", 1}, {"CG_GEMM_BK32", 1}, {"CG_WINO_BK", 0}, {"CG_NN_TILE", 0}, {"CG_TN_TILE", 0}, {"CG_NN_SPLITS", 0}, {"CG_TN_SPLITS", 0},
     {"CG_XCD_SWIZZLE", 7}, {"CG_NN_GLDS", 1}, {"CG_TN_GLDS", 1}, {"CG_WINO_GLDS", 1}, {"CG_PAD_SKIP", 20}, {"CG_WINO3", 1},
     {"CG_WINO_DGRAD_FUSE", 1}, {"CG_WINO_DGRAD_FUSE_LAUNCHES", 0}, {"CG_WINO3_LAUNCHES", 0}, {"CG_PACK_WIDE", 1},
-    {"CG_SAMPLER_ATOMIC_LAUNCHES", 0},
+    {"CG_SAMPLER_ATOMIC_LAUNCHES", 0}, {"CG_WGRAD_TAIL", 3},
 };
 long g_opt_val[OPT_COUNT];
 int g_opt_state[OPT_COUNT];
@@ -163,6 +163,7 @@
     }
     return g_opt_val[o];
 }
+bool opt_chosen(Opt o) { return g_opt_state[o] == 2 || getenv(kOptDefs[o].name) != nullptr; }
 void opt_count(Opt o) { opt(o); ++g_opt_val[o]; }
 }
 
diff --git a/cat-generator_amd/csrc/wgrad_finish.hip b/cat-generator_amd/csrc/wgrad_finish.hip
--- a/cat-generator_amd/csrc/wgrad_finish.hip
+++ b/cat-generator_amd/csrc/wgrad_finish.hip
@@ -64,10 +64,8 @@
 }
 
 template <bool UPS>
-__global__ __launch_bounds__(256) void wgrad_reduce_kernel(const float* part, float* gw, int Cin, int Cout, int k, int KK,
-                                                           int pad, int kp, int S, float scale, int CI_T, long sstride) {
-    extern __shared__ float sh[];
-    const int ci0 = blockIdx.x * CI_T, co0 = blockIdx.y * 32;
+__device__ __forceinline__ void wgrad_reduce_tile(float* sh, const float* part, float* gw, int ci0, int co0, int Cin, int Cout, int k, int KK,
+                                                  int pad, int kp, int S, float scale, int CI_T, long sstride) {
     const long plane = (long)(UPS ? kp * kp : KK) * Cin * Cout;
     const int n1 = KK * CI_T * 32;
     for (int idx = threadIdx.x; idx < n1; idx += 256) {
@@ -90,6 +88,12 @@
             *dst += scale * sh[j * 33 + co_l];
         }
     }
+}
+template <bool UPS>
+__global__ __launch_bounds__(256) void wgrad_reduce_kernel(const float* part, float* gw, int Cin, int Cout, int k, int KK,
+                                                           int pad, int kp, int S, float scale, int CI_T, long sstride) {
+    extern __shared__ float sh[];
+    wgrad_reduce_tile<UPS>(sh, part, gw, blockIdx.x * CI_T, blockIdx.y * 32, Cin, Cout, k, KK, pad, kp, S, scale, CI_T, sstride);
 }
 
 __global__ __launch_bounds__(256) void bias_part_reduce_kernel(const float* bp, float* gb, int S, int P, long sstride, int Cout, float scale) {
@@ -108,7 +112,9 @@
     float scale;
     int tr;
     int v4;
+    int ci_t;
 };
+size_t red_job_lds(const RedJob& j) { return std::max(sizeof(float) * 32 * 33, sizeof(float) * 33 * (size_t)j.KK * (size_t)j.ci_t); }
 constexpr int kRedJobs = 20;
 struct RedJobTable { RedJob j[kRedJobs]; int n; };
 
@@ -177,10 +183,16 @@
     wgrad_reduce_t_tile(t, part + (long)group * gstride, gw0 + (long)group * gws, blockIdx.x * 32, blockIdx.y * 32, Cin, Cout, S, sstride, scale);
 }
 
-__device__ __forceinline__ void red_block(float (*sh)[33], const RedJob& J, int group, int bx) {
+__device__ __forceinline__ void red_block(float* shf, const RedJob& J, int group, int bx) {
+    float (*sh)[33] = reinterpret_cast<float (*)[33]>(shf);
     if (bx >= J.wblocks) {
         float* gb = sel4(group, J.rp.gb0, J.rp.gb1, J.rp.gb2, J.rp.gb3);
         if (gb) bias_sum_block(sh, J.bias_part + (long)group * J.P * J.Cout, gb, (bx - J.wblocks) * 32, J.S, J.P, J.bsstride, J.Cout, J.scale);
+    } else if (J.ci_t) {
+        const int nci = (J.Cin + J.ci_t - 1) / J.ci_t;
+        const float* pg = J.part + (long)group * J.gstride;
+        if (J.ups) wgrad_reduce_tile<true>(shf, pg, gw_of(J.rp, group), (bx % nci) * J.ci_t, (bx / nci) * 32, J.Cin, J.Cout, J.k, J.KK, J.pad, J.kp, J.S, J.scale, J.ci_t, J.sstride);
+        else wgrad_reduce_tile<false>(shf, pg, gw_of(J.rp, group), (bx % nci) * J.ci_t, (bx / nci) * 32, J.Cin, J.Cout, J.k, J.KK, J.pad, J.kp, J.S, J.scale, J.ci_t, J.sstride);
     } else if (J.tr) {
         const int nci = J.Cin / 32;
         wgrad_reduce_t_tile(sh, J.part + (long)group * J.gstride, gw_of(J.rp, group), (bx % nci) * 32, (bx / nci) * 32, J.Cin, J.Cout, J.S, J.sstride, J.scale);
@@ -194,11 +206,12 @@
 
 __global__ __launch_bounds__(256) void wgrad_reduce_small_kernel(RedJob J) {
     __shared__ __attribute__((aligned(16))) float sh[32][33];
-    red_block(sh, J, (int)blockIdx.y, (int)blockIdx.x);
+    red_block(&sh[0][0], J, (int)blockIdx.y, (int)blockIdx.x);
 }
 
 __global__ __launch_bounds__(256) void wgrad_reduce_batch_kernel(RedJobTable t) {
-    __shared__ __attribute__((aligned(16))) float sh[32][33];
+    extern __shared__ __attribute__((aligned(16))) float sh_batch[];
+    float* sh = sh_batch;
     const int b = (int)blockIdx.x;
     int ji = 0;
     for (int q = 1; q < t.n; ++q)
@@ -251,8 +264,17 @@
 
 }
 
-int cg::wgrad_finish(hipStream_t st, const WgradParts& w, bool defer) {
-    const RedJob job = red_job(w, defer);
+static int tiled_ci_t(int KK) {
+    int ci_t = KK == 1 ? 64 : 8;
+    while (ci_t > 1 && (size_t)KK * ci_t * 33 * sizeof(float) > 60000) ci_t >>= 1;
+    return ci_t;
+}
+bool cg::wgrad_finish_tiled(int Cin, int Cout, int KK) {
+    return (long)cg::cdiv(Cin, tiled_ci_t(KK)) * cg::cdiv(Cout, 32) >= cg::kNumCU;
+}
+
+int cg::wgrad_finish(hipStream_t st, const WgradParts& w, int defer) {
+    RedJob job = red_job(w, defer != 0);
     const int Cin = w.Cin, Cout = w.Cout, KK = job.KK;
     if (w.gws && transposable(w) && !w.bias_part) {
         hipLaunchKernelGGL(wgrad_reduce_t_kernel, dim3(Cin / 32, Cout / 32, w.ngroups), dim3(256), 0, st, w.part, w.gw[0], w.gws, Cin, Cout, w.S,
@@ -260,11 +282,15 @@
         CG_LAUNCH_CHECK();
         return 0;
     }
-    int ci_t = KK == 1 ? 64 : 8;
-    while (ci_t > 1 && (size_t)KK * ci_t * 33 * sizeof(float) > 60000) ci_t >>= 1;
+    const int ci_t = tiled_ci_t(KK);
     const size_t shb = (size_t)KK * ci_t * 33 * sizeof(float);
     const dim3 rgrid(cg::cdiv(Cin, ci_t), cg::cdiv(Cout, 32));
-    if ((long)rgrid.x * rgrid.y < cg::kNumCU) return small_reduce(st, defer, job);
+    if (!wgrad_finish_tiled(Cin, Cout, KK)) return small_reduce(st, defer != 0, job);
+    if (defer == 2) {
+        job.tr = job.v4 = 0;
+        job.ci_t = ci_t; job.wblocks = (int)(rgrid.x * rgrid.y);
+        return small_reduce(st, true, job);
+    }
     for (int gi = 0; gi < w.ngroups; ++gi) {
         const float* pg = w.part + gi * job.gstride;
         float* gwi = w.gws ? w.gw[0] + gi * w.gws : w.gw[gi];
@@ -309,12 +335,14 @@
         memset(&t, 0, sizeof(t));
         t.n = (int)std::min<size_t>(kRedJobs, jobs.size() - j0);
         int blocks = 0;
+        size_t shb = 0;
         for (int q = 0; q < t.n; ++q) {
             t.j[q] = jobs[j0 + q];
             t.j[q].block0 = blocks;
             blocks += t.j[q].ngroups * (t.j[q].wblocks + t.j[q].bblocks);
+            shb = std::max(shb, red_job_lds(t.j[q]));
         }
-        hipLaunchKernelGGL(wgrad_reduce_batch_kernel, dim3(blocks), dim3(256), 0, st, t);
+        hipLaunchKernelGGL(wgrad_reduce_batch_kernel, dim3(blocks), dim3(256), shb, st, t);
         CG_LAUNCH_CHECK();
     }
     return 0;
diff --git a/include/catgan.h b/include/catgan.h
--- a/include/catgan.h
+++ b/include/catgan.h
@@ -102,6 +102,9 @@
                             float* const* gw_canonical, float* const* gb, int N, int Hp, int Wp, int Cin, int Cout,
                             int kH, int kW, int padH, int padW, int ups, float scale, void* ws, size_t ws_bytes);
 int cg_conv2d_wgrad_flush(void* stream);
+int cg_conv2d_wgrad_grouped_tail(void* stream, int ngroups, const float* const* x, const float* const* dy,
+                            float* const* gw_canonical, float* const* gb, int N, int Hp, int Wp, int Cin, int Cout,
+                            int kH, int kW, int padH, int padW, int ups, float scale, void* ws, size_t ws_bytes);
 int cg_conv2d_wgrad_gemm(void* stream, const float* x, const float* dy, int N, int Hp, int Wp, int Cin, int Cout,
                          int kH, int kW, int padH, int padW, int ups, void* ws, size_t ws_bytes);
 int cg_conv2d_wgrad_pending(void* stream, int* njobs);
```

Result: no change. 23390 (-0.2%).
